# mohammadasim98/mv-ldm

Hardware: AMD Instinct MI355X
Metric: denoised views/sec @ 256x256, 4 views, 50 DDIM steps (higher is better)
Workload: dtype bf16

## Files before the change

include/mvldm.h:

```cpp
#ifndef MVLDM_H
#define MVLDM_H

#include <stddef.h>
#include <stdint.h>

#ifdef __cplusplus
extern "C" {
#endif

#define MVLDM_ABI_VERSION 7

typedef void* mvldm_stream_t;

enum { MVLDM_F32 = 0, MVLDM_BF16 = 1, MVLDM_F16 = 2 };
enum { MVLDM_OK = 0, MVLDM_ERR_ARG = -1, MVLDM_ERR_HIP = -2, MVLDM_ERR_UNSUPPORTED = -3 };

enum { MVLDM_EPI_NONE = 0, MVLDM_EPI_SILU = 1, MVLDM_EPI_GEGLU = 2, MVLDM_EPI_GELU = 3  };
enum { MVLDM_ELT_COPY = 0, MVLDM_ELT_SILU = 1, MVLDM_ELT_GELU = 2 };

int mvldm_abi_version(void);
int mvldm_build_flags(void);
const char* mvldm_last_error(void);
int mvldm_device_info(int* cu_count, size_t* hbm_bytes, char* arch, int arch_len);

typedef struct mvldm_igemm_desc {
    const void* src0;
    const void* src1;
    const void* weight;
    const float* bias;
    const float* row_bias;
    const void* residual;
    void* dst;
    float* workspace;
    int32_t c0, c1;
    int32_t n_img, h_in, w_in, h_out, w_out;
    int32_t ksize, stride, pad, upsample;
    int32_t n_out, n_pad, k_pad;
    int32_t row_bias_ld;
    int32_t epilogue;
    int32_t act_dtype;
    int32_t dst_dtype;
    int32_t splitk;
    int32_t tile;
    int32_t k_order;
    int32_t dst_ld;
    float out_scale;
    size_t workspace_bytes;
} mvldm_igemm_desc;
int mvldm_igemm_fwd(const mvldm_igemm_desc* d, mvldm_stream_t stream);
size_t mvldm_igemm_workspace_bytes(const mvldm_igemm_desc* d);

int mvldm_pack_weight(const float* src, void* dst, int n_out, int c_in, int ksize, int c_pad, int n_pad,
                      int k_pad, int geglu, int k_order, int dst_dtype, int transpose, int c_off, int n_rows,
                      mvldm_stream_t stream);

int mvldm_pack_skinny(const void* packed, void* dst, int n_pad, int k_pad, int geglu, int dtype, mvldm_stream_t stream);
int mvldm_igemm_skinny_config(const mvldm_igemm_desc* d);

typedef struct mvldm_pack_job {
    const float* src; void* dst;
    int n_out, c_in, ksize, c_pad, n_pad, k_pad, geglu, k_order, transpose, c_off, n_rows;
    int kind;
    int blocks;
    int block0;
} mvldm_pack_job;
int mvldm_pack_job_prepare(mvldm_pack_job* job , int dst_dtype);
int mvldm_pack_weight_batch(const mvldm_pack_job* jobs , int n_jobs, const int32_t* block_job, int total_blocks,
                            int dst_dtype, mvldm_stream_t stream);

#define MVLDM_GN_MAX_CHUNKS 32
int mvldm_groupnorm_fwd(const void* x0, const void* x1, void* y, const float* gamma, const float* beta, int n_img,
                        int hw, int c0, int c1, int groups, float eps, int silu, int dtype, void* stats_ws,
                        float* stats_out, mvldm_stream_t stream);
int mvldm_groupnorm_passes(int n_img, int hw, int c, int groups, int dtype);

int mvldm_layernorm_fwd(const void* x, void* y, const float* gamma, const float* beta, int rows, int c, float eps,
                        int dtype, mvldm_stream_t stream);

int mvldm_attention_fwd(const void* q, const void* k, const void* v, void* out, int ld_q, int ld_k, int ld_v,
                        int ld_o, int heads, int head_dim, const int32_t* seg, int n_seg, int max_q_len,
                        float scale, int dtype, float* lse, int lse_ld, mvldm_stream_t stream);

int mvldm_timestep_embed_fwd(const int64_t* timesteps, const float* freqs, void* out, int n, int dim,
                             int flip_sin_to_cos, int dst_dtype, mvldm_stream_t stream);

int mvldm_eltwise_fwd(const void* x, void* y, size_t n, int op, int src_dtype, int dst_dtype, mvldm_stream_t stream);

int mvldm_ddim_cfg_step(const float* eps, const float* x_t, float* x_next, const int32_t* cond_img,
                        const int32_t* uncond_img, int n_tgt, int hw, int c, float cfg_scale, const float* coef,
                        const int32_t* step_ptr, void* unet_in, int unet_in_c, int unet_in_dtype, int n_steps,
                        float clip_range, mvldm_stream_t stream);
int mvldm_ddpm_cfg_step(const float* eps_c, const float* eps_u, const float* x_t, const float* noise, float* x_next, size_t n,
                        float cfg_scale, const float* coef, float clip_range, mvldm_stream_t stream);
int mvldm_ddim_advance(int32_t* step_ptr, const int64_t* t_table, int n_steps, int64_t* timesteps,
                       const int32_t* tgt_rows, int n_rows, mvldm_stream_t stream);

int mvldm_nchw_to_nhwc(const float* src, void* dst, int n_img, int c, int hw, int dst_c, int dst_c_off,
                       int dst_dtype, float scale, float shift, const int32_t* img_map, mvldm_stream_t stream);
int mvldm_nhwc_to_nchw(const void* src, float* dst, int n_img, int c, int hw, int src_c, int src_c_off,
                       int src_dtype, float scale, float shift, int clamp01, mvldm_stream_t stream);

enum { MVLDM_RAYS_RAW = 0, MVLDM_RAYS_POSITIONAL = 1, MVLDM_RAYS_SRT = 2 };
int mvldm_ray_channels(int mode, int n_origin_octaves, int n_dir_octaves);
int mvldm_ray_encode(const float* extrinsics, const float* intrinsics, int n_cam, int h, int w, float* out_nchw,
                     void* out_nhwc, int nhwc_c, int nhwc_c_off, int nhwc_dtype, const int32_t* img_map, int mode,
                     int n_origin_octaves, int n_dir_octaves, int plucker, mvldm_stream_t stream);

int mvldm_posterior_sample(const float* moments, const float* noise, float* out, int n, int c, int hw, float scale,
                           mvldm_stream_t stream);


typedef struct mvldm_wgrad_desc {
    const void* src0; const void* src1; const void* dy;
    float* grad;
    float* workspace; size_t workspace_bytes;
    int32_t c0, c1, c_in;
    int32_t n_img, h_in, w_in, h_out, w_out;
    int32_t ksize, stride, pad, upsample;
    int32_t n_out, dy_ld;
    int32_t act_dtype;
    int32_t accumulate;
} mvldm_wgrad_desc;
int mvldm_igemm_wgrad(const mvldm_wgrad_desc* d, mvldm_stream_t stream);

int mvldm_colsum(const void* x, float* dst, float* workspace, size_t workspace_bytes, int n_seg, int rows_per_seg, int n,
                 int ld, int ld_dst, int per_seg, int accumulate, int dtype, mvldm_stream_t stream);

#define MVLDM_NORM_BWD_STORE 0x100
int mvldm_groupnorm_bwd(const void* x0, const void* x1, const void* dy, void* dx0, void* dx1, const float* gamma,
                        const float* beta, const float* stats, float* dgamma, float* dbeta, int n_img, int hw, int c0,
                        int c1, int groups, int silu, int dtype, float* workspace, size_t workspace_bytes,
                        mvldm_stream_t stream);
int mvldm_layernorm_bwd(const void* x, const void* dy, void* dx, const float* gamma, float* dgamma, float* dbeta,
                        int rows, int c, float eps, int dtype, float* workspace, size_t workspace_bytes,
                        mvldm_stream_t stream);

typedef struct mvldm_attn_bwd_desc {
    const void* q; const void* k; const void* v; const void* out; const void* dout;
    void* dq; void* dk; void* dv;
    const float* lse; float* delta;
    const int32_t* seg;
    int32_t ld_q, ld_k, ld_v, ld_o, ld_do, ld_dq, ld_dk, ld_dv;
    int32_t heads, head_dim, n_seg, max_q_len, max_kv_len, total_q_rows, stat_ld, dtype;
    float scale;
} mvldm_attn_bwd_desc;
int mvldm_attention_bwd(const mvldm_attn_bwd_desc* d, mvldm_stream_t stream);

enum { MVLDM_TE_SILU_BWD = 0, MVLDM_TE_ADD = 1, MVLDM_TE_GEGLU_FWD = 2, MVLDM_TE_GEGLU_BWD = 3, MVLDM_TE_GELU_BWD = 4 };
int mvldm_train_eltwise(int op, const void* a, const void* b, void* out, size_t rows, int d, int a_dtype, int dtype,
                        mvldm_stream_t stream);
int mvldm_pool2x2_sum(const void* du, void* dx, int n_img, int h, int w, int c, int dtype, mvldm_stream_t stream);
int mvldm_zero_insert2x(const void* x, void* out, int n_img, int h, int w, int c, int dtype, mvldm_stream_t stream);

int mvldm_add_noise(const float* x0, const float* noise, const float* coef, void* dst, int n, int c, int hw, int dst_c,
                    int dst_c_off, int dst_dtype, const int32_t* img_map, mvldm_stream_t stream);
int mvldm_mse_loss(const float* pred, const float* noise, const int32_t* tgt_img, int n_tgt, int hw, int c, float* loss,
                   int accumulate, float loss_scale, void* dpred, int dpred_c, int dpred_dtype, float grad_scale,
                   double* workspace, mvldm_stream_t stream);

typedef struct mvldm_amp_state {
    float scale;
    int32_t growth_tracker;
    int32_t adam_step;
    int32_t found_inf;
    int32_t skipped;
    int32_t reserved[3];
} mvldm_amp_state;
int mvldm_mse_loss_amp(const float* pred, const float* noise, const int32_t* tgt_img, int n_tgt, int hw, int c, float* loss,
                       int accumulate, float loss_scale, void* dpred, int dpred_c, int dpred_dtype, float grad_scale,
                       const float* amp_scale, double* workspace, mvldm_stream_t stream);

int mvldm_grad_norm(const float* g, size_t n, const float* sumsq_in, float max_norm, float* norm_out, double* workspace,
                    mvldm_stream_t stream);
int mvldm_adamw_step(float* p, const float* g, float* m, float* v, size_t n, float lr, float beta1, float beta2, float eps,
                     float weight_decay, int step, float grad_scale, const float* clip, mvldm_stream_t stream);
int mvldm_grad_norm_amp(const float* g, size_t n, const float* sumsq_in, float max_norm, float* norm_out, mvldm_amp_state* amp,
                        double* workspace, mvldm_stream_t stream);
int mvldm_adamw_step_amp(float* p, const float* g, float* m, float* v, size_t n, float lr, float beta1, float beta2, float eps,
                         float weight_decay, float grad_scale, const float* clip, const mvldm_amp_state* amp, mvldm_stream_t stream);
int mvldm_amp_update(mvldm_amp_state* amp, float growth_factor, float backoff_factor, int growth_interval, mvldm_stream_t stream);

int mvldm_ema_update(float* avg, const float* p, size_t n, float weight, mvldm_stream_t stream);

int mvldm_gather_rows(const void* src, void* dst, const int32_t* src_index, const int32_t* dst_index, int n_rows, size_t row_bytes,
                      mvldm_stream_t stream);

int mvldm_attention_merge(const void* oa, const float* lse_a, const void* ob, const float* lse_b, void* out, const int32_t* a_img,
                          const int32_t* b_img, const int32_t* out_img, int n_img, int tokens, int heads, int head_dim, int ld_a, int ld_b,
                          int ld_o, int lse_ld_a, int lse_ld_b, int dtype, mvldm_stream_t stream);

size_t mvldm_image_metrics_workspace_bytes(int n_img, int c, int h, int w);
int mvldm_image_metrics(const float* pred, const float* gt, int n_img, int c, int h, int w, int use_sample_covariance, float* psnr,
                        float* ssim, double* workspace, size_t workspace_bytes, mvldm_stream_t stream);

size_t mvldm_lpips_workspace_bytes(int n_img, int h, int w);
int mvldm_lpips_tap_slots(int h, int w, int c);
int mvldm_lpips_prep(const float* in0, const float* in1, void* dst, int n_img, int h, int w, int c_pad, int dtype, int normalize,
                     mvldm_stream_t stream);
int mvldm_lpips_relu(void* x, size_t n, int dtype, mvldm_stream_t stream);
int mvldm_lpips_tap(const void* feat, const float* weight, void* pooled, int n_img, int h, int w, int c, int dtype, double* workspace,
                    size_t workspace_bytes, int slot0, int slots_per_image, mvldm_stream_t stream);
// ... 152 lines not shown
```

mv_ldm_amd/_build.py:

```python
from __future__ import annotations

import json
import os
import re
import subprocess
import sys
from concurrent.futures import ThreadPoolExecutor
from pathlib import Path

CSRC = Path(__file__).resolve().parent / "csrc"
LIB = CSRC / "libmvldm_hip.so"
SOURCES = ["api.cpp", "plan.cpp", "igemm.hip", "igemm_small.hip", "igemm_large.hip", "igemm_xl.hip", "igemm_halo.hip", "pack.hip", "attention.hip", "norm.hip", "misc.hip",
           "wgrad.hip", "attention_bwd.hip", "norm_bwd.hip", "train_misc.hip", "linear_pp.hip", "linear_pw.hip", "linear_ws.hip", "linear_rs.hip", "skinny.hip", "metrics.hip", "lpips.hip", "dists.hip", "fid.hip", "inception.hip", "kid.hip", "cropshim.hip", "jpeg.hip", "jpeg_host.cpp"]
HEADERS = [*sorted(CSRC.glob("*.h")), CSRC.parent.parent / "include" / "mvldm.h"]
FLAGS = ["--offload-arch=gfx950", "-O3", "-std=c++17", "-fPIC", "-ffp-contract=off", "-Wno-unused-result",
         "-Rpass-analysis=kernel-resource-usage"]
RES = CSRC / "kernel_resources.json"


def _hipcc() -> str:
    for c in (os.environ.get("HIPCC"), "/opt/rocm/bin/hipcc", "hipcc"):
        if c and (os.path.isabs(c) and os.path.exists(c) or not os.path.isabs(c)):
            return c
    raise RuntimeError("hipcc not found")


def _stale(target: Path, deps) -> bool:
    if not target.exists():
        return True
    t = target.stat().st_mtime
    return any(Path(d).stat().st_mtime > t for d in deps)


def build(force: bool = False, verbose: bool = False) -> Path:
    hipcc = _hipcc()
    flags = list(FLAGS)
    if os.environ.get("MVLDM_EXPERIMENTS") == "1":
        flags.append("-DMVLDM_EXPERIMENTS")
    objs, jobs = [], []
    for src in SOURCES:
        s = CSRC / src
        o = CSRC / (s.stem + ".o")
        objs.append(o)
        if force or _stale(o, [s, *HEADERS]):
            cmd = [hipcc, *flags, "-x", "hip", "-c", str(s), "-o", str(o)]
            jobs.append(cmd)
    if jobs:
        def run(cmd):
            if verbose:
                print(" ".join(cmd), flush=True)
            r = subprocess.run(cmd, capture_output=True, text=True)
            if r.returncode:
                raise RuntimeError(f"hipcc failed: {' '.join(cmd)}\n{r.stdout}\n{r.stderr}")
            Path(cmd[-1]).with_suffix(".res.json").write_text(json.dumps(_resources(r.stderr), indent=0))
        with ThreadPoolExecutor(max_workers=min(8, len(jobs))) as ex:
            list(ex.map(run, jobs))
    if force or jobs or _stale(LIB, objs):
        cmd = [hipcc, "--offload-arch=gfx950", "-shared", "-fPIC", "-o", str(LIB), *map(str, objs)]
        r = subprocess.run(cmd, capture_output=True, text=True)
        if r.returncode:
            raise RuntimeError(f"link failed:\n{r.stdout}\n{r.stderr}")
    parts = [o.with_suffix(".res.json") for o in objs]
    if all(q.exists() for q in parts) and (not RES.exists() or _stale(RES, parts)):
        merged = {}
        for q in parts:
            merged.update(json.loads(q.read_text()))
        RES.write_text(json.dumps(merged, indent=0, sort_keys=True))
    return LIB


_FIELDS = {"VGPRs": "vgpr", "AGPRs": "agpr", "TotalSGPRs": "sgpr", "ScratchSize [bytes/lane]": "scratch", "VGPRs Spill": "vgpr_spill",
           "Occupancy [waves/SIMD]": "waves_per_simd"}


def _resources(stderr: str) -> dict:
    out, cur = {}, None
    for line in stderr.splitlines():
        m = re.search(r"remark:\s+(.*?)\s*\[-Rpass-analysis", line)
        if not m:
            continue
        body = m.group(1)
        if body.startswith("Function Name:"):
            cur = out.setdefault(body.split(":", 1)[1].strip(), {})
        elif cur is not None and ":" in body:
            k, v = body.rsplit(":", 1)
            if k.strip() in _FIELDS and v.strip().lstrip("-").isdigit():
                cur[_FIELDS[k.strip()]] = int(v)
    return out


if __name__ == "__main__":
    print(build(force="--force" in sys.argv, verbose=True))
```

mv_ldm_amd/_lib.py:

```python
from __future__ import annotations

import ctypes as C
from pathlib import Path

LIB_PATH = Path(__file__).resolve().parent / "csrc" / "libmvldm_hip.so"

ABI_VERSION = 7
F32, BF16, F16 = 0, 1, 2
EPI_NONE, EPI_SILU, EPI_GEGLU, EPI_GELU = 0, 1, 2, 3
RAYS_RAW, RAYS_POSITIONAL, RAYS_SRT = 0, 1, 2
ELT_COPY, ELT_SILU, ELT_GELU = 0, 1, 2
NORM_BWD_STORE = 0x100
GN_MAX_CHUNKS = 32
JPEG_GRAY, JPEG_444, JPEG_422, JPEG_420 = 0, 1, 2, 3
JPEG_REASONS = ("ok", "not a JPEG", "truncated", "corrupt", "progressive", "frame type", "precision", "components", "sampling", "colour space",
                "scans", "size", "range guard")
JPEG_RANGE = 12

(OP_IGEMM, OP_GROUPNORM, OP_LAYERNORM, OP_ATTENTION, OP_TIMESTEP_EMBED, OP_ELTWISE, OP_DDIM_STEP, OP_DDIM_ADVANCE,
 OP_NCHW_TO_NHWC, OP_NHWC_TO_NCHW, OP_MEMCPY, OP_RAY_ENCODE, OP_POSTERIOR_SAMPLE,
 OP_WGRAD, OP_ATTENTION_BWD, OP_GROUPNORM_BWD, OP_LAYERNORM_BWD, OP_COLSUM, OP_TRAIN_ELTWISE, OP_POOL2X2, OP_ZERO_INSERT,
 OP_ADD_NOISE, OP_MSE_LOSS, OP_FILL_ZERO, OP_PAR_BEGIN, OP_PAR_NEXT, OP_PAR_END, OP_GATHER_ROWS, OP_ATTN_MERGE) = range(1, 30)
TE_SILU_BWD, TE_ADD, TE_GEGLU_FWD, TE_GEGLU_BWD, TE_GELU_BWD = 0, 1, 2, 3, 4

vp, i32, f32, sz = C.c_void_p, C.c_int32, C.c_float, C.c_size_t


class IgemmDesc(C.Structure):
    _fields_ = [("src0", vp), ("src1", vp), ("weight", vp), ("bias", vp), ("row_bias", vp), ("residual", vp),
                ("dst", vp), ("workspace", vp),
                ("c0", i32), ("c1", i32),
                ("n_img", i32), ("h_in", i32), ("w_in", i32), ("h_out", i32), ("w_out", i32),
                ("ksize", i32), ("stride", i32), ("pad", i32), ("upsample", i32),
                ("n_out", i32), ("n_pad", i32), ("k_pad", i32),
                ("row_bias_ld", i32), ("epilogue", i32), ("act_dtype", i32), ("dst_dtype", i32),
                ("splitk", i32), ("tile", i32), ("k_order", i32), ("dst_ld", i32), ("out_scale", f32), ("workspace_bytes", sz)]


class _GroupNorm(C.Structure):
    _fields_ = [("x", vp), ("x1", vp), ("y", vp), ("gamma", vp), ("beta", vp), ("stats_ws", vp),
                ("n_img", i32), ("hw", i32), ("c0", i32), ("c1", i32), ("groups", i32), ("silu", i32), ("dtype", i32),
                ("eps", f32), ("stats_out", vp)]


class _LayerNorm(C.Structure):
    _fields_ = [("x", vp), ("y", vp), ("gamma", vp), ("beta", vp), ("rows", i32), ("c", i32), ("dtype", i32), ("eps", f32)]


class _Attention(C.Structure):
    _fields_ = [("q", vp), ("k", vp), ("v", vp), ("out", vp), ("seg", vp),
                ("ld_q", i32), ("ld_k", i32), ("ld_v", i32), ("ld_o", i32), ("heads", i32), ("head_dim", i32),
                ("n_seg", i32), ("max_q_len", i32), ("dtype", i32), ("scale", f32), ("lse", vp), ("lse_ld", i32)]


class _Temb(C.Structure):
    _fields_ = [("timesteps", vp), ("freqs", vp), ("out", vp), ("n", i32), ("dim", i32), ("flip", i32), ("dst_dtype", i32)]


class _Eltwise(C.Structure):
    _fields_ = [("x", vp), ("y", vp), ("n", sz), ("op", i32), ("src_dtype", i32), ("dst_dtype", i32)]


class _Ddim(C.Structure):
    _fields_ = [("eps", vp), ("x_t", vp), ("x_next", vp), ("cond_img", vp), ("uncond_img", vp), ("coef", vp),
                ("step_ptr", vp), ("unet_in", vp),
                ("n_tgt", i32), ("hw", i32), ("c", i32), ("unet_in_c", i32), ("unet_in_dtype", i32), ("cfg_scale", f32),
                ("n_steps", i32), ("clip_range", f32)]


class _Advance(C.Structure):
    _fields_ = [("step_ptr", vp), ("t_table", vp), ("timesteps", vp), ("tgt_rows", vp), ("n_steps", i32), ("n_rows", i32)]


class _Layout(C.Structure):
    _fields_ = [("src", vp), ("dst", vp), ("n_img", i32), ("c", i32), ("hw", i32), ("other_c", i32),
                ("other_c_off", i32), ("dtype", i32), ("clamp01", i32), ("scale", f32), ("shift", f32), ("img_map", vp)]


class _Rays(C.Structure):
    _fields_ = [("extrinsics", vp), ("intrinsics", vp), ("out_nchw", vp), ("out_nhwc", vp), ("img_map", vp),
                ("n_cam", i32), ("h", i32), ("w", i32), ("nhwc_c", i32), ("nhwc_c_off", i32), ("nhwc_dtype", i32),
                ("mode", i32), ("n_origin_octaves", i32), ("n_dir_octaves", i32), ("plucker", i32)]


class _Posterior(C.Structure):
    _fields_ = [("moments", vp), ("noise", vp), ("out", vp), ("n", i32), ("c", i32), ("hw", i32), ("scale", f32)]


class _Memcpy(C.Structure):
    _fields_ = [("src", vp), ("dst", vp), ("bytes", sz)]


class _AttnMerge(C.Structure):
    _fields_ = [("oa", vp), ("ob", vp), ("out", vp), ("lse_a", vp), ("lse_b", vp), ("a_img", vp), ("b_img", vp), ("out_img", vp),
                ("n_img", i32), ("tokens", i32), ("heads", i32), ("head_dim", i32), ("ld_a", i32), ("ld_b", i32), ("ld_o", i32),
                ("lse_ld_a", i32), ("lse_ld_b", i32), ("dtype", i32)]


class _Gather(C.Structure):
    _fields_ = [("src", vp), ("dst", vp), ("src_index", vp), ("dst_index", vp), ("row_bytes", sz), ("n_rows", i32)]


class PackJob(C.Structure):
    _fields_ = [("src", vp), ("dst", vp), ("n_out", i32), ("c_in", i32), ("ksize", i32), ("c_pad", i32), ("n_pad", i32), ("k_pad", i32),
                ("geglu", i32), ("k_order", i32), ("transpose", i32), ("c_off", i32), ("n_rows", i32), ("kind", i32), ("blocks", i32),
                ("block0", i32)]


class WgradDesc(C.Structure):
    _fields_ = [("src0", vp), ("src1", vp), ("dy", vp), ("grad", vp), ("workspace", vp), ("workspace_bytes", sz),
                ("c0", i32), ("c1", i32), ("c_in", i32),
                ("n_img", i32), ("h_in", i32), ("w_in", i32), ("h_out", i32), ("w_out", i32),
                ("ksize", i32), ("stride", i32), ("pad", i32), ("upsample", i32),
                ("n_out", i32), ("dy_ld", i32), ("act_dtype", i32), ("accumulate", i32)]


class AttnBwdDesc(C.Structure):
    _fields_ = [("q", vp), ("k", vp), ("v", vp), ("out", vp), ("dout", vp), ("dq", vp), ("dk", vp), ("dv", vp),
                ("lse", vp), ("delta", vp), ("seg", vp),
                ("ld_q", i32), ("ld_k", i32), ("ld_v", i32), ("ld_o", i32), ("ld_do", i32), ("ld_dq", i32), ("ld_dk", i32), ("ld_dv", i32),
                ("heads", i32), ("head_dim", i32), ("n_seg", i32), ("max_q_len", i32), ("max_kv_len", i32), ("total_q_rows", i32),
                ("stat_ld", i32), ("dtype", i32), ("scale", f32)]


class _GroupNormBwd(C.Structure):
    _fields_ = [("x0", vp), ("x1", vp), ("dy", vp), ("dx0", vp), ("dx1", vp), ("gamma", vp), ("beta", vp), ("stats", vp),
                ("dgamma", vp), ("dbeta", vp), ("workspace", vp), ("workspace_bytes", sz),
                ("n_img", i32), ("hw", i32), ("c0", i32), ("c1", i32), ("groups", i32), ("silu", i32), ("dtype", i32)]


class _LayerNormBwd(C.Structure):
    _fields_ = [("x", vp), ("dy", vp), ("dx", vp), ("gamma", vp), ("dgamma", vp), ("dbeta", vp), ("workspace", vp),
                ("workspace_bytes", sz), ("rows", i32), ("c", i32), ("dtype", i32), ("eps", f32)]


class _Colsum(C.Structure):
    _fields_ = [("x", vp), ("dst", vp), ("workspace", vp), ("workspace_bytes", sz),
                ("n_seg", i32), ("rows_per_seg", i32), ("n", i32), ("ld", i32), ("ld_dst", i32), ("per_seg", i32),
                ("accumulate", i32), ("dtype", i32)]


class _TrainEltwise(C.Structure):
    _fields_ = [("a", vp), ("b", vp), ("out", vp), ("rows", sz), ("op", i32), ("d", i32), ("a_dtype", i32), ("dtype", i32)]


class _Resample(C.Structure):
    _fields_ = [("src", vp), ("dst", vp), ("n_img", i32), ("h", i32), ("w", i32), ("c", i32), ("dtype", i32)]


class _AddNoise(C.Structure):
    _fields_ = [("x0", vp), ("noise", vp), ("coef", vp), ("dst", vp), ("img_map", vp),
                ("n", i32), ("c", i32), ("hw", i32), ("dst_c", i32), ("dst_c_off", i32), ("dst_dtype", i32)]


class _Mse(C.Structure):
    _fields_ = [("pred", vp), ("noise", vp), ("tgt_img", vp), ("loss", vp), ("dpred", vp), ("workspace", vp),
                ("n_tgt", i32), ("hw", i32), ("c", i32), ("accumulate", i32), ("dpred_c", i32), ("dpred_dtype", i32),
                ("loss_scale", f32), ("grad_scale", f32), ("amp_scale", vp)]


class AmpState(C.Structure):
    _fields_ = [("scale", f32), ("growth_tracker", i32), ("adam_step", i32), ("found_inf", i32), ("skipped", i32), ("reserved", i32 * 3)]


class _Fill(C.Structure):
    _fields_ = [("dst", vp), ("bytes", sz)]
# ... 156 lines not shown
```

mv_ldm_amd/csrc/igemm.hip:

```cpp
#include <algorithm>
#include <cstdio>
#include <cstdlib>

#include "igemm_common.h"

namespace mvldm {

template <typename T> __global__ __launch_bounds__(256) void igemm_splitk_reduce(const IgemmParams p) {
    const bool geglu = p.epilogue == MVLDM_EPI_GEGLU;
    const size_t total = (size_t)p.M * p.n_dst;
    const size_t slab = (size_t)p.M * p.n_pad;
    for (size_t idx = (size_t)blockIdx.x * 256 + threadIdx.x; idx < total; idx += (size_t)gridDim.x * 256) {
        const int m = (int)(idx / p.n_dst), col = (int)(idx - (size_t)m * p.n_dst);
        float v;
        if (geglu) {
            const int nv = (col >> 5) * 64 + (col & 31), ng = nv + 32;
            float a = 0.f, g = 0.f;
            for (int s = 0; s < p.splitk; ++s) {
                a += p.ws[s * slab + (size_t)m * p.n_pad + nv];
                g += p.ws[s * slab + (size_t)m * p.n_pad + ng];
            }
            if (p.bias) { a += p.bias[col]; g += p.bias[p.n_dst + col]; }
            v = a * gelu_erf_fast(g);
        } else {
            float a = 0.f;
            for (int s = 0; s < p.splitk; ++s) a += p.ws[s * slab + (size_t)m * p.n_pad + col];
            if (p.bias) a += p.bias[col];
            if (p.row_bias) a += p.row_bias[(size_t)(m / p.hw_out) * p.row_bias_ld + col];
            if (p.epilogue == MVLDM_EPI_SILU) a = silu_f(a);
            else if (p.epilogue == MVLDM_EPI_GELU) a = gelu_erf_fast(a);
            v = a;
        }
        epilogue_store<T, true>(p, m, col, v);
    }
}

template <typename T> __global__ __launch_bounds__(256) void igemm_splitk_reduce_vec(const IgemmParams p) {
    const bool geglu = p.epilogue == MVLDM_EPI_GEGLU;
    const int cpr = p.n_dst / 8;
    const size_t total = (size_t)p.M * cpr;
    const size_t slab = (size_t)p.M * p.n_pad;
    for (size_t idx = (size_t)blockIdx.x * 256 + threadIdx.x; idx < total; idx += (size_t)gridDim.x * 256) {
        const int m = (int)(idx / cpr), col = (int)(idx - (size_t)m * cpr) * 8;
        const int nv = geglu ? (col >> 5) * 64 + (col & 31) : col;
        const float* w0 = p.ws + (size_t)m * p.n_pad + nv;
        float a[8], g[8];
#pragma unroll
        for (int e = 0; e < 8; ++e) a[e] = g[e] = 0.f;
        int s = 0;
        for (; s + 4 <= p.splitk; s += 4) {
            f32x4 lo[4], hi[4], gl[4], gh[4];
#pragma unroll
            for (int u = 0; u < 4; ++u) {
                lo[u] = *reinterpret_cast<const f32x4*>(w0 + (s + u) * slab);
                hi[u] = *reinterpret_cast<const f32x4*>(w0 + (s + u) * slab + 4);
                if (geglu) {
                    gl[u] = *reinterpret_cast<const f32x4*>(w0 + (s + u) * slab + 32);
                    gh[u] = *reinterpret_cast<const f32x4*>(w0 + (s + u) * slab + 36);
                }
            }
#pragma unroll
            for (int u = 0; u < 4; ++u) {
#pragma unroll
                for (int e = 0; e < 4; ++e) { a[e] += lo[u][e]; a[4 + e] += hi[u][e]; }
                if (geglu) {
#pragma unroll
                    for (int e = 0; e < 4; ++e) { g[e] += gl[u][e]; g[4 + e] += gh[u][e]; }
                }
            }
        }
        for (; s < p.splitk; ++s) {
            const f32x4 lo = *reinterpret_cast<const f32x4*>(w0 + s * slab), hi = *reinterpret_cast<const f32x4*>(w0 + s * slab + 4);
#pragma unroll
            for (int e = 0; e < 4; ++e) { a[e] += lo[e]; a[4 + e] += hi[e]; }
            if (geglu) {
                const f32x4 gl = *reinterpret_cast<const f32x4*>(w0 + s * slab + 32), gh = *reinterpret_cast<const f32x4*>(w0 + s * slab + 36);
#pragma unroll
                for (int e = 0; e < 4; ++e) { g[e] += gl[e]; g[4 + e] += gh[e]; }
            }
        }
        if (p.bias) {
#pragma unroll
            for (int e = 0; e < 8; ++e) a[e] += p.bias[col + e];
        }
        if (geglu) {
#pragma unroll
            for (int e = 0; e < 8; ++e) a[e] *= gelu_erf_fast(g[e] + (p.bias ? p.bias[p.n_dst + col + e] : 0.f));
        } else {
            if (p.row_bias) {
                const float* rb = p.row_bias + (size_t)(m / p.hw_out) * p.row_bias_ld + col;
#pragma unroll
                for (int e = 0; e < 8; ++e) a[e] += rb[e];
            }
            if (p.epilogue == MVLDM_EPI_SILU) {
#pragma unroll
                for (int e = 0; e < 8; ++e) a[e] = silu_f(a[e]);
            } else if (p.epilogue == MVLDM_EPI_GELU) {
#pragma unroll
                for (int e = 0; e < 8; ++e) a[e] = gelu_erf_fast(a[e]);
            }
        }
#pragma unroll
        for (int e = 0; e < 8; ++e) a[e] *= p.out_scale;
        if (p.residual) {
            const Chunk<T> rc = load_chunk<T>(reinterpret_cast<const T*>(p.residual) + (size_t)m * p.n_dst + col);
#pragma unroll
            for (int e = 0; e < 8; ++e) a[e] += rc.get(e);
        }
        size_t drow = (size_t)m;
        if (p.scatter) {
            const int img = m / p.hw_out, rem = m - img * p.hw_out;
            const int i = rem / p.w_out, j = rem - i * p.w_out;
            drow = ((size_t)img * (2 * p.h_out) + 2 * i + p.ph_y) * (size_t)(2 * p.w_out) + 2 * j + p.ph_x;
        }
        Chunk<T> oc;
#pragma unroll
        for (int e = 0; e < 8; ++e) oc.set(e, a[e]);
        store_chunk<T>(reinterpret_cast<T*>(p.dst) + drow * p.dst_ld + col, oc);
    }
}

static int env_int(const char* name, int dflt) { return knob_int(name, dflt); }
static const int kEnvTarget = env_int("MVLDM_IGEMM_TARGET", 0);
static const int kEnvSync = env_int("MVLDM_IGEMM_SYNC", 0);
static const int kEnvPx = env_int("MVLDM_IGEMM_PX", 0);
static const int kEnvNoStage = env_int("MVLDM_IGEMM_NOSTAGE", 0);
#ifdef MVLDM_EXPERIMENTS
static const int kEnvFake = env_int("MVLDM_IGEMM_FAKE", 0);
#else
static constexpr int kEnvFake = 0;
#endif

static thread_local int t_force_sync = 0;

static int launch_igemm(const IgemmParams& p, int tile, int act_dtype, hipStream_t s) {
    if (tile >= 1 && tile <= 5) return igemm_launch_small(p, tile, act_dtype, s);
    if (tile >= 6 && tile <= 8) return igemm_launch_large(p, tile, act_dtype, s);
    if (tile == 9 || tile == 10 || tile == 18) return igemm_launch_xl(p, tile, act_dtype, s);
    if (tile == 11 || tile == 17) return igemm_launch_halo(p, tile, act_dtype, s);
    return set_error(MVLDM_ERR_ARG, "igemm: bad tile %d", tile);
}


static void choose_config(const mvldm_igemm_desc& d, int M, int k_tiles, int& tile, int& splitk, size_t ws_bytes) {
    const int target = kEnvTarget ? kEnvTarget : 512;
    if (tile == 0) {
        const bool can10 = d.act_dtype != MVLDM_F32 && d.k_order == 1 && d.dst_dtype != MVLDM_F32 && d.n_pad % 320 == 0 &&
                           d.epilogue != MVLDM_EPI_GEGLU && d.upsample != 1 && d.n_out % 8 == 0 && (d.dst_ld <= 0 || d.dst_ld % 8 == 0) &&
                           !(d.ksize == 3 && d.src1);
        const int wgs10 = cdiv(M, 256) * (d.n_pad / 320);
        const double eff10 = (double)wgs10 / (256.0 * cdiv(wgs10, 256));
        if (can10 && (wgs10 >= 1024 || (wgs10 >= 512 && (eff10 >= 0.9 || d.ksize == 1)))) tile = 10;
        else if (M <= 32) tile = 5;
        else if (M <= 64) tile = 4;
        else if (d.ksize >= 2) tile = cdiv(M, 256) * cdiv(d.n_pad, 128) >= 300 ? 7 : 2;
        else if (d.n_pad >= 768 && d.act_dtype != MVLDM_F32 && d.k_order == 1 && d.dst_dtype != MVLDM_F32 &&
                 cdiv(M, 256) * cdiv(d.n_pad, 256) >= 1024)
            tile = 9;
        else if (d.k_pad >= 1024 && d.n_pad >= 1024 && cdiv(M, 128) * cdiv(d.n_pad, 256) >= 300) tile = 8;
        else tile = d.n_pad < 640 ? 2 : 3;
    }
    const int tm = cdiv(M, kTiles[tile].bm), tn = cdiv(d.n_pad, kTiles[tile].bn);
    if (splitk == 0) {
        splitk = 1;
        const int wgs = tm * tn;
        if (wgs < target) splitk = std::min(std::max(k_tiles / 4, 1), cdiv(target, wgs));
        if (d.workspace == nullptr) splitk = 1;
        while (splitk > 1 && (size_t)splitk * M * d.n_pad * sizeof(float) > ws_bytes) --splitk;
    }
    splitk = std::max(1, std::min(splitk, k_tiles));
}

static int fill_params(const mvldm_igemm_desc& d, IgemmParams& p, int& tile) {
    const int epc = d.act_dtype == MVLDM_F32 ? 4 : 8;
    const int bk = d.act_dtype == MVLDM_F32 ? 32 : 64;
    MVLDM_REQUIRE(d.src0 && d.weight && d.dst, "igemm: null pointer");
    const bool phase = d.upsample >= 2;
    MVLDM_REQUIRE(d.upsample >= 0 && d.upsample <= 5, "igemm: upsample %d", d.upsample);
    MVLDM_REQUIRE(phase ? (d.ksize == 2 && d.stride == 1 && d.h_out == d.h_in && d.w_out == d.w_in && !d.src1 && !d.residual &&
                           !d.row_bias && d.act_dtype != MVLDM_F32 && d.dst_dtype == d.act_dtype && d.k_order == 1)
                        : (d.ksize == 1 || d.ksize == 3),
                  "igemm: ksize %d / upsample %d", d.ksize, d.upsample);
    MVLDM_REQUIRE(d.stride == 1 || d.stride == 2, "igemm: stride %d", d.stride);
    MVLDM_REQUIRE(d.c0 % epc == 0 && d.c1 % epc == 0 && d.c0 > 0, "igemm: channels (%d,%d) must be multiples of %d", d.c0, d.c1, epc);
    MVLDM_REQUIRE((d.c1 == 0) == (d.src1 == nullptr), "igemm: src1/c1 mismatch");
    MVLDM_REQUIRE(d.k_pad % bk == 0 && d.k_pad >= d.ksize * d.ksize * (d.c0 + d.c1), "igemm: k_pad %d", d.k_pad);
    MVLDM_REQUIRE(d.n_pad % 64 == 0 && d.n_pad >= d.n_out, "igemm: n_pad %d (n_out %d)", d.n_pad, d.n_out);
    MVLDM_REQUIRE(d.dst_dtype == d.act_dtype || d.dst_dtype == MVLDM_F32, "igemm: dst dtype");
    if (d.epilogue == MVLDM_EPI_GEGLU)
        MVLDM_REQUIRE(d.n_out % 64 == 0 && !d.row_bias, "igemm: GEGLU needs n_out %% 64 == 0");
    p.src0 = d.src0; p.src1 = d.src1; p.weight = d.weight; p.bias = d.bias; p.row_bias = d.row_bias;
    p.residual = d.residual; p.dst = d.dst; p.ws = d.workspace;
    p.c0 = d.c0; p.c1 = d.c1; p.ctot = d.c0 + d.c1;
    p.n_img = d.n_img; p.h_in = d.h_in; p.w_in = d.w_in; p.h_out = d.h_out; p.w_out = d.w_out;
    p.hw_out = d.h_out * d.w_out;
    p.ksize = d.ksize; p.stride = d.stride; p.pad = d.pad; p.upsample = phase ? 0 : d.upsample; p.taps = d.ksize * d.ksize;
    p.scatter = phase; p.ph_y = phase ? (d.upsample - 2) >> 1 : 0; p.ph_x = phase ? (d.upsample - 2) & 1 : 0;
    p.ty0 = phase ? p.ph_y - 1 : -d.pad; p.tx0 = phase ? p.ph_x - 1 : -d.pad;
    p.cy = phase ? 1 - p.ph_y : d.ksize / 2; p.cx = phase ? 1 - p.ph_x : d.ksize / 2;
    p.M = d.n_img * p.hw_out; p.n_out = d.n_out; p.n_pad = d.n_pad; p.k_pad = d.k_pad;
    p.n_dst = d.epilogue == MVLDM_EPI_GEGLU ? d.n_out / 2 : d.n_out;
    p.rb_vec = d.row_bias && ((uintptr_t)d.row_bias % 16 == 0) && d.row_bias_ld % 4 == 0;
    p.bias_vec = d.bias && ((uintptr_t)d.bias % 16 == 0);
    p.row_bias_ld = d.row_bias_ld; p.epilogue = d.epilogue; p.dst_f32 = d.dst_dtype == MVLDM_F32;
    p.out_scale = d.out_scale;
    p.dst_ld = d.dst_ld > 0 ? d.dst_ld : p.n_dst;
    MVLDM_REQUIRE(p.dst_ld >= p.n_dst, "igemm: dst_ld %d < n_dst %d", p.dst_ld, p.n_dst);
    p.k_tiles = d.k_pad / bk;
    tile = d.tile & 63;
    t_force_sync = (d.tile >> 12) & 1;
    const int force_px = (d.tile >> 8) & 15;
    int splitk = d.splitk;
    MVLDM_REQUIRE(((tile >= 0 && tile <= kNumTiles) || tile == 17 || deep_tile(tile)) && splitk >= 0, "igemm: tile/splitk");
    choose_config(d, p.M, p.k_tiles, tile, splitk, d.workspace_bytes);
    if (splitk > 1)
        MVLDM_REQUIRE(d.workspace && (size_t)splitk * p.M * d.n_pad * sizeof(float) <= d.workspace_bytes,
                      "igemm: split-K workspace too small");
    const double es = 2.0;
    const double b0 = (double)d.n_img * d.h_in * d.w_in * d.c0 * es, b1 = (double)d.n_img * d.h_in * d.w_in * d.c1 * es;
    const double bw = (double)d.n_pad * d.k_pad * es;
    p.use_bl = d.act_dtype != MVLDM_F32 && d.k_order == 1 && !t_force_sync && !kEnvSync &&
               b0 < 4.0e9 && b1 < 4.0e9 && bw < 4.0e9;
    if (d.act_dtype != MVLDM_F32 && d.k_order == 1 && !t_force_sync && !kEnvSync && !p.use_bl) {
        static bool warned = false;
        if (!warned) {
            warned = true;
            fprintf(stderr, "[mvldm] igemm: operand of %.2f GB exceeds the 4 GB range of the fast 16-bit loop; using the slower "
                            "64-bit-address loop (split the batch to avoid this)\n", std::max(std::max(b0, b1), bw) / 1e9);
        }
    }
    p.src0_bytes = (unsigned)b0; p.src1_bytes = (unsigned)b1; p.w_bytes = (unsigned)bw;
    p.fake = kEnvFake;
    p.nt_store = stream_stores((size_t)p.M * (size_t)p.n_dst * (p.dst_f32 || d.act_dtype == MVLDM_F32 ? 4 : 2));
    if (kEnvFake & 1) p.src0_bytes = p.src1_bytes = 0;
    if (kEnvFake & 2) p.w_bytes = 0;
    if (tile >= 6 && !p.use_bl) tile = 2;
    if (deep_tile(tile) && d.upsample) tile = 2;
    p.splitk = splitk;
    if (p.use_bl) {
        const int cbs = p.k_tiles / p.taps;
        const int per = cdiv(cbs, std::min(splitk, cbs));
        p.k_tiles_per_split = per * p.taps;
        p.splitk = cdiv(cbs, per);
    } else {
        p.k_tiles_per_split = cdiv(p.k_tiles, splitk);
        p.splitk = cdiv(p.k_tiles, p.k_tiles_per_split);
    }
    p.stage_epi = d.act_dtype != MVLDM_F32 && !kEnvNoStage && (p.splitk > 1 || (!p.dst_f32 && p.n_dst % 8 == 0 && p.dst_ld % 8 == 0));
    if (tile >= 9 && tile <= 10 && (!p.stage_epi || (tile == 10 && d.epilogue == MVLDM_EPI_GEGLU))) tile = 7;
    if (tile == 11 && !(p.use_bl && p.stage_epi && p.splitk == 1 && d.ksize == 3 && d.stride == 1 && d.pad == 1 && !d.upsample &&
                        d.h_out == d.h_in && d.w_out == d.w_in && halo_rows_for(d.w_in) <= 384 && halo_smem(d.w_in) <= 160 * 1024))
        tile = 7;
    if (tile == 17 && !(p.use_bl && p.stage_epi && p.splitk == 1 && d.ksize == 3 && d.stride == 1 && d.pad == 1 && !d.upsample && d.c1 == 0 &&
                        d.h_out == d.h_in && d.w_out == d.w_in && d.epilogue != MVLDM_EPI_GEGLU && halow_smem(d.w_in) <= 160 * 1024))
        tile = 7;
    if (phase) {
        MVLDM_REQUIRE(p.use_bl && p.stage_epi, "igemm: 2x2 phase conv needs the lean 16-bit loop and an 8-aligned 16-bit output");
        if (tile != 7 && tile != 10) tile = 2;
    }
    if (p.use_bl && d.upsample == 1 && tile != 7) tile = 2;
    if (p.use_bl && d.upsample != 1) {
        const int hc = (d.h_out - 1) * d.stride + p.ty0 + p.cy, wc = (d.w_out - 1) * d.stride + p.tx0 + p.cx;
        MVLDM_REQUIRE(p.ty0 + p.cy >= 0 && p.tx0 + p.cx >= 0 && hc < d.h_in && wc < d.w_in,
                      "igemm: conv geometry (pad %d, stride %d) not supported", d.pad, d.stride);
    }
    p.tiles_m = cdiv(p.M, kTiles[tile].bm);
    p.tiles_n = cdiv(d.n_pad, kTiles[tile].bn);
    p.korder = d.k_order;
    if (d.k_order)
        MVLDM_REQUIRE(d.k_order == 1 && p.ctot % bk == 0 && d.c0 % bk == 0 && d.k_pad == p.taps * p.ctot,
                      "igemm: k_order 1 needs channel counts (%d,%d) multiples of %d", d.c0, d.c1, bk);
    {
        const double a_bytes = (double)d.n_img * d.h_in * d.w_in * p.ctot, w_bytes = (double)d.n_pad * d.k_pad;
        double best = 1e300;
        for (int px = 1; px <= 8; px *= 2) {
            const int py = 8 / px;
            const int sm = cdiv(p.tiles_m, px), sn = cdiv(p.tiles_n, py);
            const double waste = (double)(8 * sm * sn) / ((double)p.tiles_m * p.tiles_n);
            const double cost = (py * a_bytes + px * w_bytes) * waste * waste;
            if (cost < best) { best = cost; p.px = px; p.sub_m = sm; p.sub_n = sn; }
        }
        p.m_fast = w_bytes >= a_bytes;
        const int fpx = force_px ? force_px : kEnvPx;
        if (fpx > 0 && fpx <= 8 && (8 % fpx) == 0) {
            p.px = fpx; p.sub_m = cdiv(p.tiles_m, p.px); p.sub_n = cdiv(p.tiles_n, 8 / p.px);
        }
        p.grp_m = p.grp_n = 1;
        static const int kGroup = knob_int("MVLDM_IGEMM_GROUP", -1);
        if (kGroup != 0 && ((tile >= 7 && tile <= 10) || tile == 17) && p.sub_m * p.sub_n > 32) {
            const double ax = a_bytes / p.px, wx = w_bytes / (8 / p.px);
            double bestc = 1e300;
            for (int gm = 1; gm <= 32; gm *= 2) {
                if (kGroup > 0 && gm != kGroup) continue;
                const int gme = std::min(gm, p.sub_m), gne = std::min(32 / gm, p.sub_n);
                const double c = ax * cdiv(p.sub_n, gne) + wx * cdiv(p.sub_m, gme);
                if (c < bestc) { bestc = c; p.grp_m = gme; p.grp_n = gne; }
            }
        }
    }
    return MVLDM_OK;
}

int linear_pp_run(const mvldm_igemm_desc& d, hipStream_t s);
int linear_pw_run(const mvldm_igemm_desc& d, hipStream_t s);
int linear_ws_run(const mvldm_igemm_desc& d, hipStream_t s);
int skinny_run(const mvldm_igemm_desc& d, hipStream_t s);
int linear_rs_run(const mvldm_igemm_desc& d, hipStream_t s);

int igemm_run(const mvldm_igemm_desc& d, hipStream_t s) {
    IgemmParams p;
    int tile = 0;
    if (d.n_img == 0 || d.h_out == 0 || d.w_out == 0) return MVLDM_OK;
    const int req = d.tile & 63;
    if (req == 15) return skinny_run(d, s);
    if (req == 12 || req == 13 || req == 14 || req == 19) {
        MVLDM_REQUIRE(d.src0 && d.weight && d.dst, "igemm: null pointer");
        return req == 12 ? linear_pp_run(d, s) : req == 13 ? linear_pw_run(d, s) : req == 14 ? linear_ws_run(d, s) : linear_rs_run(d, s);
    }
    MVLDM_REQUIRE(d.k_order != 2, "igemm: the fragment-order pack (k_order 2) is read by tile 15 only");
    int rc = fill_params(d, p, tile);
    if (rc) return rc;
    if (p.M == 0) return MVLDM_OK;
    rc = dispatch_dtype(d.act_dtype, [&](auto t) {
        using T = decltype(t);
        int r = launch_igemm(p, tile, Elt<T>::DT, s);
        if (r) return r;
        if (p.splitk > 1) {
            if constexpr (sizeof(T) == 2) {
                if (!p.dst_f32 && p.n_dst % 8 == 0 && p.dst_ld % 8 == 0 && ((uintptr_t)p.ws % 16) == 0 &&
                    (!p.residual || ((uintptr_t)p.residual % 16) == 0) && ((uintptr_t)p.dst % 16) == 0) {
                    const size_t chunks = (size_t)p.M * (p.n_dst / 8);
                    hipLaunchKernelGGL(igemm_splitk_reduce_vec<T>, dim3((unsigned)std::min<size_t>((chunks + 255) / 256, 4096)), dim3(256), 0, s, p);
                    return check_launch();
                }
            }
            const size_t total = (size_t)p.M * p.n_dst;
            const int blocks = (int)std::min<size_t>((total + 255) / 256, 4096);
            hipLaunchKernelGGL(igemm_splitk_reduce<T>, dim3(blocks), dim3(256), 0, s, p);
            return check_launch();
        }
        return (int)MVLDM_OK;
    });
    return rc;
}

}

using namespace mvldm;

extern "C" int mvldm_igemm_fwd(const mvldm_igemm_desc* d, mvldm_stream_t stream) {
    MVLDM_REQUIRE(d != nullptr, "igemm: null desc");
    return igemm_run(*d, (hipStream_t)stream);
}

extern "C" size_t mvldm_igemm_workspace_bytes(const mvldm_igemm_desc* d) {
    if (!d) return 0;
    const size_t M = (size_t)d->n_img * d->h_out * d->w_out;
    return (size_t)16 * M * d->n_pad * sizeof(float);
}
```

mv_ldm_amd/csrc/igemm_bl.h:

```cpp
#pragma once
#include "igemm_common.h"

namespace mvldm {

template <typename T, int BM, int BN, int WM, int WN>
__global__ __launch_bounds__(WM* WN * 64) void igemm_kernel(const IgemmParams p) {
    using M_ = Mma<T>;
    constexpr int NT = WM * WN * 64;
    constexpr int EPC = Elt<T>::EPC;
    constexpr int BK = M_::BK;
    constexpr int TM = BM / WM / 32, TN = BN / WN / 32;
    constexpr int A_BYTES = BM * M_::PITCH, B_BYTES = BN * M_::PITCH;
    constexpr int A_IT = BM * 8 / NT, B_IT = BN * 8 / NT;
    static_assert(A_IT >= 1 && B_IT >= 1 && TM >= 1 && TN >= 1, "bad tile");
    extern __shared__ __attribute__((aligned(16))) char smem[];

    const int tid = threadIdx.x, lane = tid & 63, wave = tid >> 6;
    const int wm = wave / WN, wn = wave % WN;
    const int hi = lane >> 5, l31 = lane & 31;

    int split, tm, tn;
    if (!map_block(p, split, tm, tn)) return;
    const int kt0 = split * p.k_tiles_per_split;
    const int kt1 = min(kt0 + p.k_tiles_per_split, p.k_tiles);
// ... 31 lines not shown
        const bool tap_ok = tap < p.taps;
        const int ky = tap / p.ksize, kx = tap - ky * p.ksize;
        const bool from0 = c < p.c0;
        const T* sbase = from0 ? reinterpret_cast<const T*>(p.src0) + c
                               : reinterpret_cast<const T*>(p.src1) + (c - p.c0);
        const int cs = from0 ? p.c0 : p.c1;
#pragma unroll
        for (int it = 0; it < A_IT; ++it) {
            int iy = a_y[it] + ky, ix = a_x[it] + kx;
            const bool ok = tap_ok && a_img[it] >= 0 && iy >= 0 && iy < hs && ix >= 0 && ix < wsz;
            if (p.upsample) { iy >>= 1; ix >>= 1; }
            if (ok) {
                const size_t off = ((size_t)(a_img[it] * p.h_in + iy) * p.w_in + ix) * cs;
                areg[it] = *reinterpret_cast<const u32x4*>(sbase + off);
            } else {
                areg[it] = u32x4{0u, 0u, 0u, 0u};
            }
        }
#pragma unroll
        for (int it = 0; it < B_IT; ++it) {
            const int n = tn * BN + r0 + it * (NT / 8);
            if (n < p.n_pad)
                breg[it] = *reinterpret_cast<const u32x4*>(wbase + (size_t)it * (NT / 8) * p.k_pad + (size_t)kt * BK);
            else
                breg[it] = u32x4{0u, 0u, 0u, 0u};
        }
    };
    auto store_tile = [&](int stage) {
        char* at = smem + stage * (A_BYTES + B_BYTES);
        char* bt = at + A_BYTES;
#pragma unroll
        for (int it = 0; it < A_IT; ++it) M_::store(at, r0 + it * (NT / 8), kc, areg[it]);
#pragma unroll
        for (int it = 0; it < B_IT; ++it) M_::store(bt, r0 + it * (NT / 8), kc, breg[it]);
    };

    f32x16 acc[TM][TN];
#pragma unroll
    for (int i = 0; i < TM; ++i)
#pragma unroll
        for (int j = 0; j < TN; ++j)
#pragma unroll
            for (int r = 0; r < 16; ++r) acc[i][j][r] = 0.f;

    if (kt0 < kt1) {
        load_tile(kt0);
        store_tile(0);
    }
    __syncthreads();
    int cur = 0;
    for (int kt = kt0; kt < kt1; ++kt) {
        const bool more = kt + 1 < kt1;
        if (more) load_tile(kt + 1);
        const char* at = smem + cur * (A_BYTES + B_BYTES);
        const char* bt = at + A_BYTES;
#pragma unroll
        for (int kk = 0; kk < BK / M_::KI; ++kk) {
            typename M_::Frag a[TM], b[TN];
#pragma unroll
            for (int i = 0; i < TM; ++i) a[i] = M_::load(at, wm * (BM / WM) + i * 32 + l31, kk, hi);
#pragma unroll
            for (int j = 0; j < TN; ++j) b[j] = M_::load(bt, wn * (BN / WN) + j * 32 + l31, kk, hi);
#pragma unroll
            for (int i = 0; i < TM; ++i)
#pragma unroll
                for (int j = 0; j < TN; ++j) acc[i][j] = M_::mma(a[i], b[j], acc[i][j]);
        }
        if (more) store_tile(cur ^ 1);
        __syncthreads();
        cur ^= 1;
    }

    if constexpr (sizeof(T) == 2) {
        if (p.stage_epi) {
            igemm_epilogue_staged<T, BM, BN, WM, WN>(p, acc, tm, tn, split, wm, wn, wave, lane, smem);
            return;
        }
    }
    igemm_epilogue<T, BM, BN, WM, WN>(p, acc, tm, tn, split, wm, wn, hi, l31);
}


template <int TAPS, int A_IT, bool DUAL, bool UPS> struct BlAddr {
    unsigned a0[UPS ? TAPS : 1][A_IT];
    unsigned a1[DUAL ? (UPS ? TAPS : 1) : 1][DUAL ? A_IT : 1];
    unsigned mask[UPS ? 1 : A_IT];
};

template <typename T, int BM, int BN, int NW, int KS, bool DUAL, int A_IT, int B_IT, int STAGES, bool UPS, int t, int LO = 0, int HI = 1 << 20>
__device__ __forceinline__ void bl_issue(const IgemmParams& p, char* stage_base, int wave, int cb,
                                         const BlAddr<KS * KS, A_IT, DUAL, UPS>& ad, const unsigned (&vb)[B_IT]) {
    constexpr int BK = 64, TAPS = KS * KS;
    const int lead = (!UPS && KS > 1) ? p.w_in + 1 : 0;
    const int disp = UPS ? 0 : (t / KS - p.cy) * p.w_in + (t % KS - p.cx) + lead;
    const unsigned lead0 = (unsigned)lead * (unsigned)p.c0 * 2u, lead1 = (unsigned)lead * (unsigned)p.c1 * 2u;
    const __amdgpu_buffer_rsrc_t r0 = __builtin_amdgcn_make_buffer_rsrc(
        const_cast<char*>(reinterpret_cast<const char*>(p.src0)) - lead0, 0, p.src0_bytes + lead0, 0x00020000);
    const __amdgpu_buffer_rsrc_t r1 = __builtin_amdgcn_make_buffer_rsrc(
        const_cast<char*>(reinterpret_cast<const char*>(DUAL ? p.src1 : p.src0)) - (DUAL ? lead1 : lead0), 0,
        DUAL ? p.src1_bytes + lead1 : p.src0_bytes + lead0, 0x00020000);
    const __amdgpu_buffer_rsrc_t rw = __builtin_amdgcn_make_buffer_rsrc(const_cast<void*>(p.weight), 0, p.w_bytes, 0x00020000);
    char* at = stage_base;
    char* bt = at + BM * 128;
    const int c = cb * BK;
    const bool from0 = !DUAL || c < p.c0;
    const int soff = ((from0 ? c : c - p.c0) + disp * (from0 ? p.c0 : p.c1)) * 2;
#pragma unroll
    for (int it = (LO > 0 ? LO : 0); it < (HI < A_IT ? HI : A_IT); ++it) {
        __attribute__((address_space(3))) void* dst = (__attribute__((address_space(3))) void*)(at + (wave + NW * it) * 1024);
        unsigned v0, v1;
        if constexpr (UPS) {
            v0 = ad.a0[t][it];
            v1 = ad.a1[DUAL ? t : 0][DUAL ? it : 0];
        } else {
            const bool ok = (ad.mask[it] >> t) & 1u;
            v0 = ok ? ad.a0[0][it] : kBufOob;
            v1 = ok ? ad.a1[0][DUAL ? it : 0] : kBufOob;
        }
        if (from0) __builtin_amdgcn_raw_ptr_buffer_load_lds(r0, dst, 16, v0, soff, 0, 0);
        else __builtin_amdgcn_raw_ptr_buffer_load_lds(r1, dst, 16, v1, soff, 0, 0);
    }
    const int koff = (cb * TAPS + t) * (BK * 2);
#pragma unroll
    for (int it = (LO > A_IT ? LO - A_IT : 0); it < (HI - A_IT < B_IT ? HI - A_IT : B_IT); ++it)
        __builtin_amdgcn_raw_ptr_buffer_load_lds(rw, (__attribute__((address_space(3))) void*)(bt + (wave + NW * it) * 1024), 16,
                                                 vb[it], koff, 0, 0);
}

template <typename T, int BM, int BN, int WM, int WN>
__device__ __forceinline__ void bl_compute(const char* stage_base, f32x16 (&acc)[BM / WM / 32][BN / WN / 32], int wm, int wn,
                                           int hi, int l31) {
    constexpr int TM = BM / WM / 32, TN = BN / WN / 32;
#pragma unroll
    for (int kk = 0; kk < 64 / Mma<T>::KI; ++kk) {
        BlFrags<T, TM, TN> f;
        bl_load<T, BM, BN, WM, WN>(stage_base, f, kk, wm, wn, hi, l31);
        bl_mma<T, TM, TN>(f, acc);
    }
}

template <int LPT, int MAXY>
__device__ __forceinline__ void bl_wait_young(int young) {
    if constexpr (MAXY >= 1) {
        if (young >= MAXY) {
            asm volatile("s_waitcnt vmcnt(%0) lgkmcnt(0)" ::"n"(MAXY * LPT) : "memory");
            return;
        }
        bl_wait_young<LPT, MAXY - 1>(young);
    } else {
        asm volatile("s_waitcnt vmcnt(0) lgkmcnt(0)" ::: "memory");
    }
}

template <typename T, int BM, int BN, int WM, int WN, int KS, bool DUAL, int STAGES, bool UPS>
__global__ __launch_bounds__(WM* WN * 64) void igemm_bl_kernel(const IgemmParams p) {
    using M_ = Mma<T>;
    static_assert(sizeof(T) == 2, "16-bit activation types only");
    constexpr int NW = WM * WN, TAPS = KS * KS;
    constexpr int BK = 64, EPC = 8;
    constexpr int TM = BM / WM / 32, TN = BN / WN / 32;
    constexpr int A_BYTES = BM * 128, B_BYTES = BN * 128, STAGE_BYTES = A_BYTES + B_BYTES;
    constexpr int A_IT = BM / 8 / NW, B_IT = BN / 8 / NW, LPT = A_IT + B_IT;
    static_assert(A_IT >= 1 && B_IT >= 1 && (BM / 8) % NW == 0 && (BN / 8) % NW == 0, "bad tile");
    static_assert(STAGES >= 2 && STAGES <= 8, "ring depth");
    extern __shared__ __attribute__((aligned(16))) char smem[];

    const auto [lane, wave, wm, wn, hi, l31] = wave_lane<WN>();
    int split, tm, tn;
    if (!map_block(p, split, tm, tn)) return;
    const int cb0 = split * (p.k_tiles_per_split / TAPS);
    const int cb1 = min(cb0 + p.k_tiles_per_split / TAPS, p.k_tiles / TAPS);

    const int slot = lane & 7, rsub = lane >> 3;
    BlAddr<TAPS, A_IT, DUAL, UPS> ad;
#pragma unroll
    for (int it = 0; it < A_IT; ++it) {
        const int row = (wave + NW * it) * 8 + rsub;
        const int m = tm * BM + row;
        const unsigned chunk = (unsigned)((slot ^ ((row >> 1) & 7)) * EPC);
        const bool live = m < p.M;
        const int img = live ? m / p.hw_out : 0, rem = live ? m - img * p.hw_out : 0;
        const int oy = rem / p.w_out, ox = rem - oy * p.w_out;
        if constexpr (UPS) {
            const unsigned hs = 2 * p.h_in, wsz = 2 * p.w_in;
            const int y0 = live ? oy * p.stride - p.pad : -(1 << 20), x0 = ox * p.stride - p.pad;
#pragma unroll
            for (int t = 0; t < TAPS; ++t) {
                const int iy = y0 + t / KS, ix = x0 + t % KS;
                const bool ok = (unsigned)iy < hs && (unsigned)ix < wsz;
                const unsigned pix = (unsigned)(img * p.h_in + (iy >> 1)) * (unsigned)p.w_in + (unsigned)(ix >> 1);
                ad.a0[t][it] = ok ? (pix * (unsigned)p.c0 + chunk) * 2u : kBufOob;
                if constexpr (DUAL) ad.a1[t][it] = ok ? (pix * (unsigned)p.c1 + chunk) * 2u : kBufOob;
            }
        } else {
            const int yc = oy * p.stride + p.ty0 + p.cy, xc = ox * p.stride + p.tx0 + p.cx;
            const unsigned pix = (unsigned)(img * p.h_in + yc) * (unsigned)p.w_in + (unsigned)xc;
            unsigned msk = 0;
#pragma unroll
            for (int t = 0; t < TAPS; ++t) {
                const int iy = yc + t / KS - p.cy, ix = xc + t % KS - p.cx;
                msk |= (live && (unsigned)iy < (unsigned)p.h_in && (unsigned)ix < (unsigned)p.w_in) ? (1u << t) : 0u;
            }
            ad.a0[0][it] = (pix * (unsigned)p.c0 + chunk) * 2u;
            if constexpr (DUAL) ad.a1[0][it] = (pix * (unsigned)p.c1 + chunk) * 2u;
            ad.mask[it] = msk;
        }
    }
    unsigned vb[B_IT];
#pragma unroll
    for (int it = 0; it < B_IT; ++it) {
        const int row = (wave + NW * it) * 8 + rsub;
        const int n = tn * BN + row;
        const unsigned chunk = (unsigned)((slot ^ ((row >> 1) & 7)) * EPC);
        vb[it] = n < p.n_pad ? ((unsigned)n * (unsigned)p.k_pad + chunk) * 2u : kBufOob;
    }

    f32x16 acc[TM][TN];
#pragma unroll
    for (int i = 0; i < TM; ++i)
#pragma unroll
        for (int j = 0; j < TN; ++j)
#pragma unroll
            for (int r = 0; r < 16; ++r) acc[i][j][r] = 0.f;

#define MVLDM_BL_ISSUE(stage_, cb_, t_) \
    bl_issue<T, BM, BN, NW, KS, DUAL, A_IT, B_IT, STAGES, UPS, t_>(p, smem + (stage_) * STAGE_BYTES, wave, cb_, ad, vb)
#define MVLDM_BL_ISSUE_R(stage_, cb_, t_, lo_, hi_) \
    bl_issue<T, BM, BN, NW, KS, DUAL, A_IT, B_IT, STAGES, UPS, t_, lo_, hi_>(p, smem + (stage_) * STAGE_BYTES, wave, cb_, ad, vb)
#define MVLDM_BL_NEXT(t_, d_) (((t_) + (d_)) % TAPS)
#define MVLDM_BL_LOAD(f_, slot_, kk_) bl_load<T, BM, BN, WM, WN>(smem + (slot_) * STAGE_BYTES, f_, kk_, wm, wn, hi, l31)
#define MVLDM_BL_MMA(f_)                  \
    __builtin_amdgcn_sched_barrier(0);    \
    bl_mma<T, TM, TN>(f_, acc);           \
    __builtin_amdgcn_sched_barrier(0);
#define MVLDM_BL_STEP(t_)                                                                                         \
    {                                                                                                             \
        static_assert(64 / M_::KI == 4, "four k-sub-steps per K-tile");                                          \
        MVLDM_BL_LOAD(f1, slot_c, 1);                                                                             \
        MVLDM_BL_MMA(f0)                                                                                          \
        MVLDM_BL_LOAD(f0, slot_c, 2);                                                                             \
        MVLDM_BL_MMA(f1)                                                                                          \
        MVLDM_BL_LOAD(f1, slot_c, 3);                                                                             \
        MVLDM_BL_MMA(f0)                                                                                          \
            \
                             \
        if (STAGES == 3 && cb + ((t_) + 2) / TAPS < cb1) asm volatile("s_waitcnt vmcnt(%0) lgkmcnt(0)" ::"n"(LPT) : "memory"); \
        else asm volatile("s_waitcnt vmcnt(0) lgkmcnt(0)" ::: "memory");                                          \
        __builtin_amdgcn_s_barrier();                                                                             \
        {                                                                                                         \
                   \
            const int cbn_ = cb + ((t_) + STAGES) / TAPS;                                                         \
            if (cbn_ < cb1) { MVLDM_BL_ISSUE(slot_c, cbn_, MVLDM_BL_NEXT(t_, STAGES)); }                          \
        }                                                                                                         \
        slot_c = slot_c + 1 == STAGES ? 0 : slot_c + 1;                                                           \
        MVLDM_BL_LOAD(f0, slot_c, 0);                                                                             \
        MVLDM_BL_MMA(f1)                                                                                          \
    }
#ifdef MVLDM_BL_BURST
    constexpr bool SPREAD_S = false;
#elif defined(MVLDM_BL_SPREAD_ALL)
    constexpr bool SPREAD_S = true;
#else
    constexpr bool SPREAD_S = NW == 8;
#endif
#define MVLDM_BL_STEP_SIMPLE(t_)                                                                                  \
    {                                                                                                             \
        asm volatile("s_waitcnt vmcnt(0) lgkmcnt(0)" ::: "memory");                                               \
        __builtin_amdgcn_s_barrier();                                                                             \
        if constexpr (!SPREAD_S) {                                                                                \
            const int cbn_ = cb + ((t_) + 1) / TAPS;                                                              \
            if (cbn_ < cb1) { MVLDM_BL_ISSUE(slot_c ^ 1, cbn_, MVLDM_BL_NEXT(t_, 1)); }                           \
            bl_compute<T, BM, BN, WM, WN>(smem + slot_c * STAGE_BYTES, acc, wm, wn, hi, l31);                     \
        } else {                                                                                                  \
            constexpr int Q0_ = (4 * LPT + 8) / 9, Q1_ = Q0_ + (LPT - Q0_ + 1) / 2;                              \
            const int cbn_ = cb + ((t_) + 1) / TAPS;                                                              \
            const bool more_ = cbn_ < cb1;                                                                        \
            if (more_) { MVLDM_BL_ISSUE_R(slot_c ^ 1, cbn_, MVLDM_BL_NEXT(t_, 1), 0, Q0_); }                      \
            {                                                                                                     \
                BlFrags<T, TM, TN> fs_;                                                                           \
                MVLDM_BL_LOAD(fs_, slot_c, 0);                                                                    \
                bl_mma<T, TM, TN>(fs_, acc);                                                                      \
            }                                                                                                     \
            if (more_) { MVLDM_BL_ISSUE_R(slot_c ^ 1, cbn_, MVLDM_BL_NEXT(t_, 1), Q0_, Q1_); }                    \
            {                                                                                                     \
                BlFrags<T, TM, TN> fs_;                                                                           \
                MVLDM_BL_LOAD(fs_, slot_c, 1);                                                                    \
                bl_mma<T, TM, TN>(fs_, acc);                                                                      \
            }                                                                                                     \
            if (more_) { MVLDM_BL_ISSUE_R(slot_c ^ 1, cbn_, MVLDM_BL_NEXT(t_, 1), Q1_, LPT); }                    \
            {                                                                                                     \
                BlFrags<T, TM, TN> fs_;                                                                           \
                MVLDM_BL_LOAD(fs_, slot_c, 2);                                                                    \
                bl_mma<T, TM, TN>(fs_, acc);                                                                      \
                MVLDM_BL_LOAD(fs_, slot_c, 3);                                                                    \
                bl_mma<T, TM, TN>(fs_, acc);                                                                      \
            }                                                                                                     \
        }                                                                                                         \
        slot_c ^= 1;                                                                                              \
    }
#define MVLDM_BL_STEP_DEEP(t_)                                                                                    \
    {                                                                                                             \
        bl_wait_young<LPT, STAGES - 2>((cb1 - cb) * TAPS - (t_) - 1);       \
        __builtin_amdgcn_s_barrier();                                       \
        {                                                                                                         \
            const int cbn_ = cb + ((t_) + STAGES - 1) / TAPS;                                                     \
            if (cbn_ < cb1) { MVLDM_BL_ISSUE(slot_c == 0 ? STAGES - 1 : slot_c - 1, cbn_, MVLDM_BL_NEXT(t_, STAGES - 1)); } \
        }                                                                                                         \
        bl_compute<T, BM, BN, WM, WN>(smem + slot_c * STAGE_BYTES, acc, wm, wn, hi, l31);                         \
        slot_c = slot_c + 1 == STAGES ? 0 : slot_c + 1;                                                           \
    }
#define MVLDM_BL_PRO(j_)                                                                                          \
    if constexpr (STAGES - 1 > (j_)) {                                                                            \
        if (cb0 + (j_) / TAPS < cb1) { MVLDM_BL_ISSUE((j_), cb0 + (j_) / TAPS, ((j_) % TAPS)); }                  \
    }
    constexpr bool PIPE = NW == 8 && TM * TN <= 8 && STAGES <= 3;
    if constexpr (STAGES > 3) {
        static_assert((STAGES - 2) * LPT <= 63, "vmcnt is a 6-bit counter");
        if (cb0 < cb1) {
            MVLDM_BL_ISSUE(0, cb0, 0);
            MVLDM_BL_PRO(1) MVLDM_BL_PRO(2) MVLDM_BL_PRO(3) MVLDM_BL_PRO(4) MVLDM_BL_PRO(5) MVLDM_BL_PRO(6)
            int slot_c = 0;
            for (int cb = cb0; cb < cb1; ++cb) {
                MVLDM_BL_STEP_DEEP(0)
                if constexpr (TAPS == 4) { MVLDM_BL_STEP_DEEP(1) MVLDM_BL_STEP_DEEP(2) MVLDM_BL_STEP_DEEP(3) }
                if constexpr (TAPS == 9) {
                    MVLDM_BL_STEP_DEEP(1) MVLDM_BL_STEP_DEEP(2) MVLDM_BL_STEP_DEEP(3) MVLDM_BL_STEP_DEEP(4)
                    MVLDM_BL_STEP_DEEP(5) MVLDM_BL_STEP_DEEP(6) MVLDM_BL_STEP_DEEP(7) MVLDM_BL_STEP_DEEP(8)
                }
            }
        }
    } else if constexpr (!PIPE) {
        static_assert(STAGES == 2, "the plain loop uses the 2-slot ring");
        if (cb0 < cb1) {
            MVLDM_BL_ISSUE(0, cb0, 0);
            int slot_c = 0;
            for (int cb = cb0; cb < cb1; ++cb) {
                MVLDM_BL_STEP_SIMPLE(0)
                if constexpr (TAPS == 4) { MVLDM_BL_STEP_SIMPLE(1) MVLDM_BL_STEP_SIMPLE(2) MVLDM_BL_STEP_SIMPLE(3) }
                if constexpr (TAPS == 9) {
                    MVLDM_BL_STEP_SIMPLE(1) MVLDM_BL_STEP_SIMPLE(2) MVLDM_BL_STEP_SIMPLE(3) MVLDM_BL_STEP_SIMPLE(4)
                    MVLDM_BL_STEP_SIMPLE(5) MVLDM_BL_STEP_SIMPLE(6) MVLDM_BL_STEP_SIMPLE(7) MVLDM_BL_STEP_SIMPLE(8)
                }
            }
        }
    } else if (cb0 < cb1) {
        MVLDM_BL_ISSUE(0, cb0, 0);
        const bool has1 = cb0 + 1 / TAPS < cb1, has2 = STAGES == 3 && cb0 + 2 / TAPS < cb1;
        if (has1) { MVLDM_BL_ISSUE(1, cb0 + 1 / TAPS, (1 % TAPS)); }
        if constexpr (STAGES == 3) {
            if (has2) { MVLDM_BL_ISSUE(2, cb0 + 2 / TAPS, (2 % TAPS)); }
        }
        if (has2) asm volatile("s_waitcnt vmcnt(%0)" ::"n"(2 * LPT) : "memory");
        else if (has1) asm volatile("s_waitcnt vmcnt(%0)" ::"n"(LPT) : "memory");
        else asm volatile("s_waitcnt vmcnt(0)" ::: "memory");
        __builtin_amdgcn_s_barrier();
        int slot_c = 0;
        BlFrags<T, TM, TN> f0, f1;
        MVLDM_BL_LOAD(f0, 0, 0);
        for (int cb = cb0; cb < cb1; ++cb) {
            MVLDM_BL_STEP(0)
            if constexpr (TAPS == 4) { MVLDM_BL_STEP(1) MVLDM_BL_STEP(2) MVLDM_BL_STEP(3) }
            if constexpr (TAPS == 9) {
                MVLDM_BL_STEP(1) MVLDM_BL_STEP(2) MVLDM_BL_STEP(3) MVLDM_BL_STEP(4)
                MVLDM_BL_STEP(5) MVLDM_BL_STEP(6) MVLDM_BL_STEP(7) MVLDM_BL_STEP(8)
            }
        }
    }
#undef MVLDM_BL_STEP_SIMPLE
#undef MVLDM_BL_STEP_DEEP
#undef MVLDM_BL_PRO
#undef MVLDM_BL_LOAD
#undef MVLDM_BL_MMA
#undef MVLDM_BL_NEXT
#undef MVLDM_BL_STEP
#undef MVLDM_BL_ISSUE
#undef MVLDM_BL_ISSUE_R
    asm volatile("s_waitcnt vmcnt(0)" ::: "memory");
    if constexpr (TM * TN > 4) {
        igemm_epilogue_staged<T, BM, BN, WM, WN>(p, acc, tm, tn, split, wm, wn, wave, lane, smem);
    } else {
        if (p.stage_epi) igemm_epilogue_staged<T, BM, BN, WM, WN>(p, acc, tm, tn, split, wm, wn, wave, lane, smem);
        else igemm_epilogue<T, BM, BN, WM, WN>(p, acc, tm, tn, split, wm, wn, hi, l31);
    }
}

template <typename T, int BM, int BN, int WM, int WN> static int launch_sync(const IgemmParams& p, hipStream_t s) {
    static std::atomic<uint64_t> done{0};
    constexpr int ring = 2 * (BM + BN) * Mma<T>::PITCH, park = WM * WN * 32 * (park_blocks(BN / WN / 32) * 32 + 4) * 4;
    return launch_kernel(igemm_kernel<T, BM, BN, WM, WN>, done, (sizeof(T) == 2 && park > ring) ? park : ring,
                         8 * p.sub_m * p.sub_n * p.splitk, WM * WN * 64, p, s);
}

template <typename T, int BM, int BN, int WM, int WN, int KS, bool DUAL, int STAGES, bool UPS>
static int launch_bl_s(const IgemmParams& p, hipStream_t s) {
    static std::atomic<uint64_t> done{0};
    constexpr int ring = STAGES * (BM + BN) * 128, park = WM * WN * 32 * (park_blocks(BN / WN / 32) * 32 + 4) * 4;
    return launch_kernel(igemm_bl_kernel<T, BM, BN, WM, WN, KS, DUAL, STAGES, UPS>, done, ring > park ? ring : park,
                         8 * p.sub_m * p.sub_n * p.splitk, WM * WN * 64, p, s);
}
template <typename T, int BM, int BN, int WM, int WN, int KS, bool DUAL, int DEPTH = 0>
static int launch_bl(const IgemmParams& p, hipStream_t s) {
    constexpr int STAGES = DEPTH ? DEPTH : ((WM * WN == 8 && 3 * (BM + BN) * 128 <= 160 * 1024) ? 3 : 2);
    if (p.upsample) {
        if constexpr (KS == 3 && !DUAL && ((BM == 128 && BN == 64) || (BM == 256 && BN == 128)))
            return launch_bl_s<T, BM, BN, WM, WN, KS, DUAL, STAGES, true>(p, s);
        else
            return set_error(MVLDM_ERR_ARG, "igemm: upsampling 3x3 conv needs tile 2 or 7 on the 16-bit path");
    }
    return launch_bl_s<T, BM, BN, WM, WN, KS, DUAL, STAGES, false>(p, s);
}
template <typename T, int BM, int BN, int WM, int WN, int DEPTH> static int launch_bl_deep(const IgemmParams& p, hipStream_t s) {
    const bool dual = p.c1 > 0;
    if (p.ksize == 3) return dual ? launch_bl<T, BM, BN, WM, WN, 3, true, DEPTH>(p, s) : launch_bl<T, BM, BN, WM, WN, 3, false, DEPTH>(p, s);
    if (p.ksize == 1) return dual ? launch_bl<T, BM, BN, WM, WN, 1, true, DEPTH>(p, s) : launch_bl<T, BM, BN, WM, WN, 1, false, DEPTH>(p, s);
    return set_error(MVLDM_ERR_ARG, "igemm: the deep-ring tiles take 1x1 and 3x3 convs");
}

template <typename T, int BM, int BN, int WM, int WN> static int launch_bl_any(const IgemmParams& p, hipStream_t s) {
    const bool dual = p.c1 > 0;
    if (p.ksize == 2) {
        if constexpr ((BM == 128 && BN == 64) || (BM == 256 && BN == 128) || (BM == 256 && BN == 320))
            return launch_bl<T, BM, BN, WM, WN, 2, false>(p, s);
        else
            return set_error(MVLDM_ERR_ARG, "igemm: 2x2 phase conv needs tile 2, 7 or 10");
    }
    if (p.ksize == 3) {
        if (!dual) return launch_bl<T, BM, BN, WM, WN, 3, false>(p, s);
        if constexpr (BM == 256 && BN >= 256)
            return set_error(MVLDM_ERR_UNSUPPORTED, "igemm: tiles 9 / 10 do not take a two-source 3x3 conv (use tile 7 or 11)");
        else
            return launch_bl<T, BM, BN, WM, WN, 3, true>(p, s);
    }
    return dual ? launch_bl<T, BM, BN, WM, WN, 1, true>(p, s) : launch_bl<T, BM, BN, WM, WN, 1, false>(p, s);
}

template <typename T, int BM, int BN, int WM, int WN> static int launch_tile(const IgemmParams& p, hipStream_t s) {
    if constexpr (sizeof(T) == 2) {
        if (p.use_bl) return launch_bl_any<T, BM, BN, WM, WN>(p, s);
    }
    return launch_sync<T, BM, BN, WM, WN>(p, s);
}

}
```

mv_ldm_amd/csrc/igemm_common.h:

```cpp
#pragma once
#include <algorithm>

#include "common.h"

namespace mvldm {

struct IgemmParams {
    const void* src0; const void* src1; const void* weight;
    const float* bias; const float* row_bias; const void* residual; void* dst; float* ws;
    int c0, c1, ctot;
    int n_img, h_in, w_in, h_out, w_out, hw_out;
    int ksize, stride, pad, upsample;
    int M, n_out, n_pad, n_dst, k_pad, taps;
    int row_bias_ld, epilogue, dst_f32, dst_ld;
    float out_scale;
    int splitk, k_tiles, k_tiles_per_split;
    int tiles_m, tiles_n;
    int korder;
    int px, sub_m, sub_n, m_fast;
    int grp_m, grp_n;
    int rb_vec;
    int bias_vec;
    int ty0, tx0, cy, cx;
    int scatter, ph_y, ph_x;
    int fake;
    unsigned src0_bytes, src1_bytes, w_bytes;
    int use_bl, stage_epi;
    int nt_store;
};

template <typename T> struct Mma;

template <typename T16> struct Mma16 : Mfma16<T16> {
    static constexpr int KI = 16;
    static constexpr int BK = 64;
    static constexpr int PITCH = 128;
    using Frag = typename Mfma16<T16>::Frag;
    static __device__ __forceinline__ void store(char* tile, int r, int kc, u32x4 v) {
        *reinterpret_cast<u32x4*>(tile + r * PITCH + ((kc ^ ((r >> 1) & 7)) << 4)) = v;
    }
    static __device__ __forceinline__ Frag load(const char* tile, int r, int kk, int hi) {
        const int kc = kk * 2 + hi;
        return *reinterpret_cast<const Frag*>(tile + r * PITCH + ((kc ^ ((r >> 1) & 7)) << 4));
    }
};
template <> struct Mma<bf16_t> : Mma16<bf16_t> {};
template <> struct Mma<f16_t> : Mma16<f16_t> {};
template <> struct Mma<float> {
    static constexpr int KI = 2;
    static constexpr int BK = 32;
    static constexpr int PITCH = 33 * 4;
    using Frag = float;
    static __device__ __forceinline__ void store(char* tile, int r, int kc, u32x4 v) {
        uint32_t* p = reinterpret_cast<uint32_t*>(tile + r * PITCH + kc * 16);
        p[0] = v[0]; p[1] = v[1]; p[2] = v[2]; p[3] = v[3];
    }
    static __device__ __forceinline__ Frag load(const char* tile, int r, int kk, int hi) {
        return *reinterpret_cast<const float*>(tile + r * PITCH + (kk * 2 + hi) * 4);
    }
    static __device__ __forceinline__ f32x16 mma(Frag a, Frag b, f32x16 c) {
        return __builtin_amdgcn_mfma_f32_32x32x2f32(a, b, c, 0, 0, 0);
    }
};

__device__ __forceinline__ int orig_col(int n_packed, int n_out, bool geglu) {
    if (!geglu) return n_packed;
    const int blk = n_packed >> 5, w = n_packed & 31;
    return (blk & 1) ? (n_out >> 1) + (blk >> 1) * 32 + w : (blk >> 1) * 32 + w;
}

template <typename T, bool SCATTER = false>
__device__ __forceinline__ void epilogue_store(const IgemmParams& p, int m, int n_dst_col, float v) {
    v *= p.out_scale;
    if (p.residual) v += to_f32<T>(reinterpret_cast<const T*>(p.residual)[(size_t)m * p.n_dst + n_dst_col]);
    size_t drow = (size_t)m;
    if (SCATTER && p.scatter) {
        const int img = m / p.hw_out, rem = m - img * p.hw_out;
        const int i = rem / p.w_out, j = rem - i * p.w_out;
        drow = ((size_t)img * (2 * p.h_out) + 2 * i + p.ph_y) * (size_t)(2 * p.w_out) + 2 * j + p.ph_x;
    }
    const size_t o = drow * p.dst_ld + n_dst_col;
    if (p.dst_f32) reinterpret_cast<float*>(p.dst)[o] = v;
    else reinterpret_cast<T*>(p.dst)[o] = from_f32<T>(v);
}

__device__ __forceinline__ bool map_block(const IgemmParams& p, int& split, int& tm, int& tn) {
    const int b = blockIdx.x, xcd = b & 7, idx = b >> 3;
    const int xm = xcd % p.px, xn = xcd / p.px;
    const int per = p.sub_m * p.sub_n;
    split = idx / per;
    const int r = idx - split * per;
    int tml, tnl;
    if (p.grp_m * p.grp_n > 1) {
        const int gm = p.grp_m, gn = p.grp_n;
        const int nfull = p.sub_m / gm, per_super = gm * p.sub_n;
        int mg, gm_eff, rr;
        if (r < nfull * per_super) { mg = r / per_super; rr = r - mg * per_super; gm_eff = gm; }
        else { mg = nfull; rr = r - nfull * per_super; gm_eff = p.sub_m - nfull * gm; }
        const int ng = rr / (gm_eff * gn), r2 = rr - ng * gm_eff * gn;
        tnl = ng * gn + r2 / gm_eff;
        tml = mg * gm + r2 % gm_eff;
    } else if (p.m_fast) { tnl = r / p.sub_m; tml = r - tnl * p.sub_m; }
    else { tml = r / p.sub_n; tnl = r - tml * p.sub_n; }
    tm = xm * p.sub_m + tml;
    tn = xn * p.sub_n + tnl;
    return tm < p.tiles_m && tn < p.tiles_n;
}

template <typename T, int BM, int BN, int WM, int WN>
__device__ __forceinline__ void igemm_epilogue(const IgemmParams& p, f32x16 (&acc)[BM / WM / 32][BN / WN / 32], int tm, int tn,
                                               int split, int wm, int wn, int hi, int l31) {
    constexpr int TM = BM / WM / 32, TN = BN / WN / 32;
    const bool geglu = p.epilogue == MVLDM_EPI_GEGLU;
    if (p.splitk > 1) {
        float* ws = p.ws + (size_t)split * p.M * p.n_pad;
#pragma unroll
        for (int i = 0; i < TM; ++i)
#pragma unroll
            for (int j = 0; j < TN; ++j) {
                const int n = tn * BN + wn * (BN / WN) + j * 32 + l31;
#pragma unroll
                for (int r = 0; r < 16; ++r) {
                    const int m = tm * BM + wm * (BM / WM) + i * 32 + (r & 3) + 8 * (r >> 2) + 4 * hi;
                    if (m < p.M && n < p.n_pad) ws[(size_t)m * p.n_pad + n] = acc[i][j][r];
                }
            }
        return;
    }
#pragma unroll
    for (int i = 0; i < TM; ++i) {
        if (geglu) {
            if constexpr (TN % 2 == 0) {
#pragma unroll
                for (int j = 0; j < TN; j += 2) {
                    const int nb = tn * BN + wn * (BN / WN) + j * 32;
                    const int col = (nb >> 6) * 32 + l31;
                    if (col >= p.n_dst) continue;
                    const float bv = p.bias ? p.bias[col] : 0.f;
                    const float bg = p.bias ? p.bias[p.n_dst + col] : 0.f;
#pragma unroll
                    for (int r = 0; r < 16; ++r) {
                        const int m = tm * BM + wm * (BM / WM) + i * 32 + (r & 3) + 8 * (r >> 2) + 4 * hi;
                        if (m >= p.M) continue;
                        epilogue_store<T>(p, m, col, (acc[i][j][r] + bv) * gelu_erf_fast(acc[i][j + 1][r] + bg));
                    }
                }
            }
        } else {
#pragma unroll
            for (int j = 0; j < TN; ++j) {
                const int n = tn * BN + wn * (BN / WN) + j * 32 + l31;
                if (n >= p.n_out) continue;
                const float bv = p.bias ? p.bias[n] : 0.f;
#pragma unroll
                for (int r = 0; r < 16; ++r) {
                    const int m = tm * BM + wm * (BM / WM) + i * 32 + (r & 3) + 8 * (r >> 2) + 4 * hi;
                    if (m >= p.M) continue;
                    float v = acc[i][j][r] + bv;
                    if (p.row_bias) v += p.row_bias[(size_t)(m / p.hw_out) * p.row_bias_ld + n];
                    if (p.epilogue == MVLDM_EPI_SILU) v = silu_f(v);
                    else if (p.epilogue == MVLDM_EPI_GELU) v = gelu_erf_fast(v);
                    epilogue_store<T>(p, m, n, v);
                }
            }
        }
    }
}

constexpr int park_blocks(int tn) { return tn <= 4 ? tn : 4; }

enum { EPI_PLAIN = 0, EPI_ACT_SILU = 1, EPI_PAIR_GEGLU = 2, EPI_PARTIAL = 3, EPI_ACT_GELU = 4 };

template <typename T, int JN, int MODE, int PITCH>
__device__ __forceinline__ void epi_rows(const IgemmParams& p, const float* st, int m0, int pcol0, int split, int lane) {
    constexpr bool PAIR = MODE == EPI_PAIR_GEGLU;
    constexpr int WC = PAIR ? JN * 16 : JN * 32;
    constexpr int CPR = WC / 8;
    static_assert(64 % CPR == 0 && (32 * CPR) % 64 == 0, "row-major mapping");
    constexpr int RSTEP = 64 / CPR, ITERS = 32 / RSTEP;
    const int ch = lane % CPR, row0 = lane / CPR;
    const int ncol0 = PAIR ? (pcol0 >> 1) : pcol0;
// ... 17 lines not shown
            }
        } else {
#pragma unroll
            for (int e = 0; e < 8; ++e) {
                bv[e] = p.bias[n0 + e];
                if constexpr (PAIR) bg[e] = p.bias[p.n_dst + n0 + e];
            }
        }
    }
    const bool rb_on = MODE != EPI_PARTIAL && MODE != EPI_PAIR_GEGLU && p.row_bias != nullptr;
    Chunk<T> rpre[ITERS];
    if constexpr (MODE != EPI_PARTIAL) {
        if (p.residual && !(p.fake & 4)) {
#pragma unroll
            for (int it = 0; it < ITERS; ++it) {
                const int m = m0 + row0 + it * RSTEP;
                if (m < p.M) rpre[it] = load_chunk<T>(reinterpret_cast<const T*>(p.residual) + (size_t)m * p.n_dst + n0);
            }
        }
    }
    float rbv[8];
    bool rb_pre = false;
    if (rb_on) {
        const int img0 = m0 / p.hw_out;
        rb_pre = p.rb_vec && (min(m0 + 31, p.M - 1) / p.hw_out) == img0;
        if (rb_pre) {
            const float* rb = p.row_bias + (size_t)img0 * p.row_bias_ld + n0;
            const f32x4 r0 = *reinterpret_cast<const f32x4*>(rb), r1 = *reinterpret_cast<const f32x4*>(rb + 4);
#pragma unroll
            for (int e = 0; e < 4; ++e) { rbv[e] = r0[e]; rbv[4 + e] = r1[e]; }
        }
    }
#pragma unroll
    for (int it = 0; it < ITERS; ++it) {
        const int row = row0 + it * RSTEP;
        const int m = m0 + row;
        if (m >= p.M) continue;
        const f32x4 a = *reinterpret_cast<const f32x4*>(st + row * PITCH + voff);
        const f32x4 b = *reinterpret_cast<const f32x4*>(st + row * PITCH + voff + 4);
        if constexpr (MODE == EPI_PARTIAL) {
            float* o = p.ws + (size_t)split * p.M * p.n_pad + (size_t)m * p.n_pad + n0;
            *reinterpret_cast<f32x4*>(o) = a;
            *reinterpret_cast<f32x4*>(o + 4) = b;
        } else {
            float v[8] = {a[0] + bv[0], a[1] + bv[1], a[2] + bv[2], a[3] + bv[3], b[0] + bv[4], b[1] + bv[5], b[2] + bv[6], b[3] + bv[7]};
            if constexpr (PAIR) {
                const f32x4 ga = *reinterpret_cast<const f32x4*>(st + row * PITCH + voff + 32);
                const f32x4 gb = *reinterpret_cast<const f32x4*>(st + row * PITCH + voff + 36);
#pragma unroll
                for (int e = 0; e < 4; ++e) {
                    v[e] *= gelu_erf_16(ga[e] + bg[e]);
                    v[4 + e] *= gelu_erf_16(gb[e] + bg[4 + e]);
                }
            } else {
                if (rb_on && rb_pre) {
#pragma unroll
                    for (int e = 0; e < 8; ++e) v[e] += rbv[e];
                } else if (rb_on) {
                    const float* rb = p.row_bias + (size_t)(m / p.hw_out) * p.row_bias_ld + n0;
                    if (p.rb_vec) {
                        const f32x4 r0 = *reinterpret_cast<const f32x4*>(rb), r1 = *reinterpret_cast<const f32x4*>(rb + 4);
#pragma unroll
                        for (int e = 0; e < 4; ++e) { v[e] += r0[e]; v[4 + e] += r1[e]; }
                    } else {
#pragma unroll
                        for (int e = 0; e < 8; ++e) v[e] += rb[e];
                    }
                }
                if constexpr (MODE == EPI_ACT_SILU) {
#pragma unroll
                    for (int e = 0; e < 8; ++e) v[e] = silu_f(v[e]);
                }
                if constexpr (MODE == EPI_ACT_GELU) {
#pragma unroll
                    for (int e = 0; e < 8; ++e) v[e] = gelu_erf_fast(v[e]);
                }
            }
#pragma unroll
            for (int e = 0; e < 8; ++e) v[e] *= p.out_scale;
            if (p.fake & 4) { if (v[0] == 1.2345e33f) p.ws[0] = v[1]; continue; }
            if (p.residual) {
#pragma unroll
                for (int e = 0; e < 8; ++e) v[e] += rpre[it].get(e);
            }
            Chunk<T> oc;
#pragma unroll
            for (int e = 0; e < 8; ++e) oc.set(e, v[e]);
            size_t drow = (size_t)m;
            if (p.scatter) {
                const int img = m / p.hw_out, rem = m - img * p.hw_out;
                const int i = rem / p.w_out, j = rem - i * p.w_out;
                drow = ((size_t)img * (2 * p.h_out) + 2 * i + p.ph_y) * (size_t)(2 * p.w_out) + 2 * j + p.ph_x;
            }
            T* const dptr = reinterpret_cast<T*>(p.dst) + drow * p.dst_ld + n0;
            if (p.nt_store) __builtin_nontemporal_store(oc.raw, reinterpret_cast<u32x4*>(dptr));
            else store_chunk<T>(dptr, oc);
        }
    }
}

template <int TM, int TN, int I, int J0, int JN, int PITCH>
__device__ __forceinline__ void epi_park(const f32x16 (&acc)[TM][TN], float* st, int lane) {
    const int hi = lane >> 5, l31 = lane & 31;
#pragma unroll
    for (int j = 0; j < JN; ++j)
#pragma unroll
        for (int r = 0; r < 16; ++r) st[((r & 3) + 8 * (r >> 2) + 4 * hi) * PITCH + j * 32 + l31] = acc[I][J0 + j][r];
}

template <typename T, int JN, int PITCH>
__device__ __forceinline__ void epi_group_rows(const IgemmParams& p, const float* st, int m0, int pcol0, int split, int mode, int lane) {
    if (mode == EPI_PARTIAL) epi_rows<T, JN, EPI_PARTIAL, PITCH>(p, st, m0, pcol0, split, lane);
    else if (mode == EPI_PAIR_GEGLU) {
        if constexpr (JN % 2 == 0) epi_rows<T, JN, EPI_PAIR_GEGLU, PITCH>(p, st, m0, pcol0, split, lane);
    } else if (mode == EPI_ACT_SILU) epi_rows<T, JN, EPI_ACT_SILU, PITCH>(p, st, m0, pcol0, split, lane);
    else if (mode == EPI_ACT_GELU) epi_rows<T, JN, EPI_ACT_GELU, PITCH>(p, st, m0, pcol0, split, lane);
    else epi_rows<T, JN, EPI_PLAIN, PITCH>(p, st, m0, pcol0, split, lane);
}

template <typename T, int BM, int BN, int WM, int WN, int I>
__device__ __forceinline__ void igemm_epilogue_rowblock(const IgemmParams& p, const f32x16 (&acc)[BM / WM / 32][BN / WN / 32], float* st, int tm, int tn,
                                                        int split, int wm, int wn, int mode, int lane) {
    constexpr int TM = BM / WM / 32, TN = BN / WN / 32;
    constexpr int WCOLS = BN / WN;
    constexpr int JG = park_blocks(TN);
    constexpr int PITCH = JG * 32 + 4;
    const int m0 = tm * BM + wm * (BM / WM) + I * 32;
    const int pcol0 = tn * BN + wn * WCOLS;
    epi_park<TM, TN, I, 0, JG, PITCH>(acc, st, lane);
    epi_group_rows<T, JG, PITCH>(p, st, m0, pcol0, split, mode, lane);
    if constexpr (TN > JG) {
        epi_park<TM, TN, I, JG, TN - JG, PITCH>(acc, st, lane);
        epi_group_rows<T, TN - JG, PITCH>(p, st, m0, pcol0 + JG * 32, split, mode, lane);
    }
    if constexpr (I + 1 < TM) igemm_epilogue_rowblock<T, BM, BN, WM, WN, I + 1>(p, acc, st, tm, tn, split, wm, wn, mode, lane);
}

template <typename T, int BM, int BN, int WM, int WN>
__device__ __forceinline__ void igemm_epilogue_staged(const IgemmParams& p, f32x16 (&acc)[BM / WM / 32][BN / WN / 32], int tm,
                                                      int tn, int split, int wm, int wn, int wave, int lane, char* smem) {
    constexpr int TN = BN / WN / 32;
    constexpr int JG = park_blocks(TN);
    constexpr int PITCH = JG * 32 + 4;
    static_assert(TN <= 2 * JG, "at most two park groups");
    if (p.fake & 8) return;
    float* st = reinterpret_cast<float*>(smem) + wave * (32 * PITCH);
    const int mode = p.splitk > 1 ? EPI_PARTIAL
                                  : (p.epilogue == MVLDM_EPI_GEGLU ? EPI_PAIR_GEGLU
                                     : (p.epilogue == MVLDM_EPI_SILU ? EPI_ACT_SILU : (p.epilogue == MVLDM_EPI_GELU ? EPI_ACT_GELU : EPI_PLAIN)));
    __syncthreads();
    igemm_epilogue_rowblock<T, BM, BN, WM, WN, 0>(p, acc, st, tm, tn, split, wm, wn, mode, lane);
}

struct WaveLane { int lane, wave, wm, wn, hi, l31; };
template <int WN> __device__ __forceinline__ WaveLane wave_lane() {
    const int tid = threadIdx.x, lane = tid & 63;
    const int wave = __builtin_amdgcn_readfirstlane(tid >> 6);
    return {lane, wave, wave / WN, wave % WN, lane >> 5, lane & 31};
}

template <typename T, int TM, int TN> struct BlFrags {
    typename Mma<T>::Frag a[TM], b[TN];
};

template <typename T, int BM, int BN, int WM, int WN>
__device__ __forceinline__ void bl_load(const char* stage_base, BlFrags<T, BM / WM / 32, BN / WN / 32>& f, int kk, int wm, int wn,
                                        int hi, int l31) {
    using M_ = Mma<T>;
    constexpr int TM = BM / WM / 32, TN = BN / WN / 32;
    const char* at = stage_base;
    const char* bt = at + BM * 128;
#pragma unroll
    for (int i = 0; i < TM; ++i) f.a[i] = M_::load(at, wm * (BM / WM) + i * 32 + l31, kk, hi);
#pragma unroll
    for (int j = 0; j < TN; ++j) f.b[j] = M_::load(bt, wn * (BN / WN) + j * 32 + l31, kk, hi);
}

template <typename T, int TM, int TN>
__device__ __forceinline__ void bl_mma(const BlFrags<T, TM, TN>& f, f32x16 (&acc)[TM][TN]) {
#pragma unroll
    for (int i = 0; i < TM; ++i)
#pragma unroll
        for (int j = 0; j < TN; ++j) acc[i][j] = Mma<T>::mma(f.a[i], f.b[j], acc[i][j]);
}

inline int cdiv(int a, int b) { return (a + b - 1) / b; }
struct TileCfg { int bm, bn, threads; };
constexpr TileCfg kTiles[] = {{0, 0, 0}, {128, 128, 256}, {128, 64, 256}, {64, 128, 256}, {64, 64, 128}, {32, 64, 64},
                                 {256, 64, 256},
                                 {256, 128, 512},
                                 {128, 256, 512},
                                 {256, 256, 512},
                                 {256, 320, 512},
                                 {256, 128, 512},
                                 {0, 0, 0}, {0, 0, 0}, {0, 0, 0}, {0, 0, 0},
                                 {0, 0, 0},
                                 {256, 320, 512},
                                 {192, 128, 512}};
constexpr int kNumTiles = 11;
inline bool deep_tile(int tile) { return tile == 18; }

template <typename KernT> inline int launch_kernel(KernT kern, std::atomic<uint64_t>& attr_done, int smem, int blocks, int threads,
                                                   const IgemmParams& p, hipStream_t s) {
    if (int rc0 = ensure_dyn_smem(reinterpret_cast<const void*>(kern), smem, attr_done)) return rc0;
    hipLaunchKernelGGL(kern, dim3(blocks), dim3(threads), smem, s, p);
    return check_launch();
}

inline int halo_rows_for(int w_in) { return (256 + 2 * (w_in + 1) + 7) / 8 * 8; }
inline int halo_smem(int w_in) { return 2 * halo_rows_for(w_in) * 128 + 3 * 128 * 128 + 128 + 1024; }
inline int halow_smem(int w_in) { return 2 * halo_rows_for(w_in) * 128 + 2 * 320 * 128 + 128 + 1024; }

inline int require_bl(const IgemmParams& p, int tile, int act_dtype) {
    if (act_dtype != MVLDM_F32 && p.use_bl) return MVLDM_OK;
    return set_error(MVLDM_ERR_ARG, "igemm: tile %d needs the 16-bit block-major path", tile);
}
template <typename F> inline int dispatch_16bit(int dtype, F&& f) { return dtype == MVLDM_BF16 ? f(bf16_t{}) : f(f16_t{}); }

int igemm_launch_small(const IgemmParams& p, int tile, int act_dtype, hipStream_t s);
int igemm_launch_large(const IgemmParams& p, int tile, int act_dtype, hipStream_t s);
int igemm_launch_xl(const IgemmParams& p, int tile, int act_dtype, hipStream_t s);
int igemm_launch_halo(const IgemmParams& p, int tile, int act_dtype, hipStream_t s);

}
```

mv_ldm_amd/ops.py:

```python
from __future__ import annotations

import ctypes as C
import os
from dataclasses import dataclass
from typing import NamedTuple, Optional, Sequence

import math

import numpy as np
import torch

from . import _lib as L

_DT = {torch.float32: L.F32, torch.bfloat16: L.BF16, torch.float16: L.F16}


def dt(t) -> int:
    return _DT[t if isinstance(t, torch.dtype) else t.dtype]


def epc(dtype: torch.dtype) -> int:
    return 4 if dtype == torch.float32 else 8


# ... 39 lines not shown
            and self.ksize in (1, 2, 3) and self.n_out % 4 == 0

    def skinny(self) -> torch.Tensor:
        if self._skinny is None:
            assert self.can_skinny(), "tile 15 needs a 16-bit block-major pack with channels in multiples of 64"
            out = torch.empty_like(self.data)
            L.check(L.load().mvldm_pack_skinny(self.data.data_ptr(), out.data_ptr(), self.n_pad, self.k_pad, int(self.geglu), dt(self.data), stream()))
            self._skinny = out
        return self._skinny

    def drop_skinny(self):
        if not self._skinny_pinned:
            self._skinny = None


def block_k(dtype: torch.dtype) -> int:
    return 32 if dtype == torch.float32 else 64


def pack_weight_t(w: torch.Tensor, dtype: torch.dtype, c_off: int = 0, n_rows: Optional[int] = None,
                  out: Optional[torch.Tensor] = None) -> PackedWeight:
    assert w.is_cuda and w.dtype == torch.float32 and w.is_contiguous()
    n_out, c_in = w.shape[0], w.shape[1]
    ksize = w.shape[2] if w.ndim == 4 else 1
    n_rows = c_in - c_off if n_rows is None else n_rows
    c_pad = _roundup(n_out, epc(dtype))
    bk = block_k(dtype)
    k_pad = _roundup(ksize * ksize * c_pad, bk)
    n_pad = _roundup(n_rows, 64)
    k_order = int(c_pad % bk == 0)
    data = torch.zeros(n_pad, k_pad, dtype=dtype, device=w.device) if out is None else out
    L.check(L.load().mvldm_pack_weight(w.data_ptr(), data.data_ptr(), n_out, c_in, ksize, c_pad, n_pad, k_pad, 0, k_order, dt(dtype),
                                       1, c_off, n_rows, stream()))
    return PackedWeight(data, n_rows, n_pad, k_pad, c_pad, ksize, False, k_order)


def pack_weight(w: torch.Tensor, dtype: torch.dtype, c_pad: Optional[int] = None, geglu: bool = False,
                c_split: Optional[int] = None, out: Optional[torch.Tensor] = None) -> PackedWeight:
    assert w.is_cuda, "pack_weight needs a device tensor (no CPU path)"
    w = w.detach().to(torch.float32).contiguous()
    n_out, c_in = w.shape[0], w.shape[1]
    ksize = w.shape[2] if w.ndim == 4 else 1
    e = epc(dtype)
    c_pad = _roundup(c_in, e) if c_pad is None else c_pad
    bk = block_k(dtype)
    k_pad = _roundup(ksize * ksize * c_pad, bk)
    n_pad = _roundup(n_out, 64)
    k_order = int(c_pad % bk == 0 and (c_split is None or c_split % bk == 0))
    out = torch.empty(n_pad, k_pad, dtype=dtype, device=w.device) if out is None else out
    L.check(L.load().mvldm_pack_weight(w.data_ptr(), out.data_ptr(), n_out, c_in, ksize, c_pad, n_pad, k_pad,
                                       int(geglu), k_order, dt(dtype), 0, 0, n_out, stream()))
    return PackedWeight(out, n_out, n_pad, k_pad, c_pad, ksize, geglu, k_order)


def pack_job(w: torch.Tensor, pw: PackedWeight, *, transpose: bool = False, c_off: int = 0) -> "L.PackJob":
    assert w.is_cuda and w.dtype == torch.float32 and w.is_contiguous()
    j = L.PackJob()
    j.src, j.dst = w.data_ptr(), pw.data.data_ptr()
    j.n_out, j.c_in, j.ksize = w.shape[0], w.shape[1], pw.ksize
    j.c_pad, j.n_pad, j.k_pad, j.geglu, j.k_order = pw.c_pad, pw.n_pad, pw.k_pad, int(pw.geglu), pw.k_order
    j.transpose, j.c_off, j.n_rows = int(transpose), c_off, (pw.n_out if transpose else w.shape[0])
    L.check(L.load().mvldm_pack_job_prepare(C.byref(j), dt(pw.data.dtype)))
    return j


class PackBatch:

    def __init__(self, jobs: Sequence["L.PackJob"], dtype: torch.dtype, device):
        self.n, self.dtype = len(jobs), dtype
        arr = (L.PackJob * max(len(jobs), 1))()
        b0 = 0
        for i, j in enumerate(jobs):
            C.memmove(C.byref(arr[i]), C.byref(j), C.sizeof(L.PackJob))
            arr[i].block0 = b0
            b0 += j.blocks
        self.total_blocks = b0
        raw = torch.frombuffer(bytearray(bytes(arr)), dtype=torch.uint8).clone()
        self.table = raw.to(device)
        self.block_job = None
        if jobs:
            self.block_job = torch.repeat_interleave(torch.arange(len(jobs), dtype=torch.int32), torch.tensor([j.blocks for j in jobs])).to(device)
            assert self.block_job.numel() == b0

    def run(self):
        L.check(L.load().mvldm_pack_weight_batch(self.table.data_ptr(), self.n, None if self.block_job is None else self.block_job.data_ptr(),
                                                 self.total_blocks, dt(self.dtype), stream()))


def conv_out_hw(h: int, w: int, ksize: int, stride: int, pad: int, upsample) -> tuple:
    if int(upsample) >= 2:
        return h, w
    hs, ws = (2 * h, 2 * w) if upsample else (h, w)
    if ksize == 3 and stride == 2 and pad == 0:
        return (hs + 1 - 3) // 2 + 1, (ws + 1 - 3) // 2 + 1
    return (hs + 2 * pad - ksize) // stride + 1, (ws + 2 * pad - ksize) // stride + 1


def use_skinny(d, pw: PackedWeight) -> torch.Tensor:
    t = pw.skinny()
    d.weight, d.k_order = ptr(t), 2
    return t


def igemm_desc(src0, src1, pw: PackedWeight, dst, *, n_img, h_in, w_in, h_out, w_out, stride=1, pad=None, upsample=False,
               bias=None, row_bias=None, residual=None, epilogue=L.EPI_NONE, out_scale=1.0, ws=None, splitk=0,
               tile=0, into=None) -> L.IgemmDesc:
    d = L.IgemmDesc() if into is None else into
    c0 = src0.shape[-1]
    c1 = 0 if src1 is None else src1.shape[-1]
    assert c0 + c1 == pw.c_pad, f"weight packed for {pw.c_pad} channels, sources give {c0}+{c1}"
    assert not pw.k_order or c0 % block_k(src0.dtype) == 0, "weight packed block-major but the source split is unaligned"
    d.src0, d.src1, d.weight = ptr(src0), ptr(src1), ptr(pw.data)
    d.bias, d.row_bias, d.residual, d.dst = ptr(bias), ptr(row_bias), ptr(residual), ptr(dst)
    d.c0, d.c1 = c0, c1
    d.n_img, d.h_in, d.w_in, d.h_out, d.w_out = n_img, h_in, w_in, h_out, w_out
    d.ksize, d.stride, d.upsample = pw.ksize, stride, int(upsample)
    d.pad = (pw.ksize // 2) if pad is None else pad
    d.n_out, d.n_pad, d.k_pad = pw.n_out, pw.n_pad, pw.k_pad
    d.row_bias_ld = 0 if row_bias is None else row_bias.stride(0)
    d.epilogue, d.act_dtype, d.dst_dtype = epilogue, dt(src0), dt(dst)
    d.splitk, d.tile, d.out_scale = splitk, tile, out_scale
    n_dst = pw.n_out // 2 if epilogue == L.EPI_GEGLU else pw.n_out
    d.dst_ld = 0 if dst.shape[-1] == n_dst else dst.shape[-1]
    d.k_order = pw.k_order
    if (tile & 63) == 15:
        use_skinny(d, pw)
    if ws is not None:
        d.workspace, d.workspace_bytes = ws.data_ptr(), ws.numel() * ws.element_size()
    else:
        d.workspace, d.workspace_bytes = None, 0
        if splitk == 0:
            d.splitk = 1
    return d


def conv2d(x: torch.Tensor, pw: PackedWeight, bias=None, *, x2=None, stride=1, pad=None, upsample=False, row_bias=None,
           residual=None, epilogue=L.EPI_NONE, out_dtype=None, out_scale=1.0, splitk=0, tile=0, out=None, dst=None) -> torch.Tensor:
    assert x.is_cuda and x.is_contiguous() and (x2 is None or x2.is_contiguous())
    n, h, w, _ = x.shape
    pad = (pw.ksize // 2) if pad is None else pad
    ho, wo = conv_out_hw(h, w, pw.ksize, stride, pad, upsample)
    n_dst = pw.n_out // 2 if epilogue == L.EPI_GEGLU else pw.n_out
    if dst is not None:
        up = 2 if int(upsample) >= 2 else 1
        assert out is None and dst.is_contiguous() and dst.dtype == (out_dtype or x.dtype) and dst.shape[-1] > n_dst
        assert dst.numel() == n * up * ho * up * wo * dst.shape[-1]
        out = dst
    elif out is None:
        out = torch.empty(n, ho, wo, n_dst, dtype=out_dtype or x.dtype, device=x.device)
    else:
        assert out.is_contiguous() and out.numel() == n * ho * wo * n_dst and out.dtype == (out_dtype or x.dtype)
        out = out.view(n, ho, wo, n_dst)
    scratch = None
    if splitk != 1:
        scratch = workspace(min(16 * n * ho * wo * pw.n_pad * 4, 256 << 20), x.device)
    d = igemm_desc(x, x2, pw, out, n_img=n, h_in=h, w_in=w, h_out=ho, w_out=wo, stride=stride, pad=pad,
                   upsample=upsample, bias=bias, row_bias=row_bias, residual=residual, epilogue=epilogue,
                   out_scale=out_scale, ws=scratch, splitk=splitk, tile=tile)
    L.check(L.load().mvldm_igemm_fwd(C.byref(d), stream()))
    return out


def upsample_phase_weights(w: torch.Tensor) -> list:
    assert w.ndim == 4 and w.shape[2:] == (3, 3)
    w = w.detach().to(torch.float32)
    rows = {0: (w[:, :, 0], w[:, :, 1] + w[:, :, 2]), 1: (w[:, :, 0] + w[:, :, 1], w[:, :, 2])}
    out = []
    for py in (0, 1):
        for px in (0, 1):
            taps = []
            for r in rows[py]:
                cols = (r[:, :, 0], r[:, :, 1] + r[:, :, 2]) if px == 0 else (r[:, :, 0] + r[:, :, 1], r[:, :, 2])
                taps.append(torch.stack(cols, dim=-1))
            out.append(torch.stack(taps, dim=-2).contiguous())
    return out


def conv2d_upsample_phases(x: torch.Tensor, pws, bias=None, tile=0, splitk=0) -> torch.Tensor:
    n, h, w, _ = x.shape
    out = torch.empty(n, 2 * h, 2 * w, pws[0].n_out, dtype=x.dtype, device=x.device)
    scratch = workspace(min(16 * n * h * w * pws[0].n_pad * 4, 256 << 20), x.device)
    for phase, pw in enumerate(pws):
        d = igemm_desc(x, None, pw, out, n_img=n, h_in=h, w_in=w, h_out=h, w_out=w, stride=1, pad=0, upsample=2 + phase,
                       bias=bias, splitk=splitk, tile=tile, ws=scratch)
        L.check(L.load().mvldm_igemm_fwd(C.byref(d), stream()))
    return out


def linear(x: torch.Tensor, pw: PackedWeight, bias=None, *, residual=None, epilogue=L.EPI_NONE, out_dtype=None,
           splitk=0, tile=0, out=None, dst=None) -> torch.Tensor:
    rows, c = x.shape
    y = conv2d(x.view(rows, 1, 1, c), pw, bias, residual=None if residual is None else residual.view(rows, 1, 1, -1),
               epilogue=epilogue, out_dtype=out_dtype, splitk=splitk, tile=tile, out=out, dst=None if dst is None else dst.view(rows, 1, 1, -1))
    return y.view(rows, -1)


def groupnorm(x: torch.Tensor, gamma, beta, groups: int, eps: float, silu: bool, x2=None, stats_out=None, out=None) -> torch.Tensor:
    assert x.is_cuda and x.is_contiguous() and (x2 is None or x2.is_contiguous())
    n, c0 = x.shape[0], x.shape[-1]
    c1 = 0 if x2 is None else x2.shape[-1]
    hw = math.prod(x.shape[1:-1])
    if out is None:
        y = torch.empty(*x.shape[:-1], c0 + c1, dtype=x.dtype, device=x.device)
    else:
        assert out.is_contiguous() and out.dtype == x.dtype and out.numel() == n * hw * (c0 + c1)
        y = out.view(*x.shape[:-1], c0 + c1)
    ws = workspace(max(n, 1) * L.GN_MAX_CHUNKS * groups * 2 * 8, x.device, "gn")
    L.check(L.load().mvldm_groupnorm_fwd(x.data_ptr(), ptr(x2), y.data_ptr(), gamma.data_ptr(), beta.data_ptr(), n, hw, c0, c1,
                                         groups, eps, int(silu), dt(x), ws.data_ptr(), ptr(stats_out), stream()))
    return y


def layernorm(x: torch.Tensor, gamma, beta, eps: float = 1e-5, out=None) -> torch.Tensor:
    assert x.is_cuda and x.is_contiguous()
    c = x.shape[-1]
    rows = x.numel() // c
    if out is None:
        y = torch.empty_like(x)
    else:
        assert out.is_contiguous() and out.dtype == x.dtype and out.numel() == x.numel()
        y = out.view(x.shape)
    L.check(L.load().mvldm_layernorm_fwd(x.data_ptr(), y.data_ptr(), gamma.data_ptr(), beta.data_ptr(), rows, c, eps,
                                         dt(x), stream()))
    return y


def make_segments(q_lens, kv_lens=None, device="cuda") -> torch.Tensor:
    kv_lens = q_lens if kv_lens is None else kv_lens
    rows, q0, k0 = [], 0, 0
    for ql, kl in zip(q_lens, kv_lens):
        rows.append([q0, ql, k0, kl])
        q0, k0 = q0 + ql, k0 + kl
    return torch.tensor(rows, dtype=torch.int32, device=device)


def attention(q: torch.Tensor, k: torch.Tensor, v: torch.Tensor, heads: int, head_dim: int, seg: torch.Tensor,
              max_q_len: int, scale: Optional[float] = None, lse: Optional[torch.Tensor] = None, out=None) -> torch.Tensor:
    assert q.is_cuda and q.stride(1) == 1 and k.stride(1) == 1 and v.stride(1) == 1
    if out is None:
        out = torch.empty(q.shape[0], heads * head_dim, dtype=q.dtype, device=q.device)
    assert out.stride(1) == 1 and out.dtype == q.dtype and out.shape[1] == heads * head_dim
    scale = head_dim ** -0.5 if scale is None else scale
    L.check(L.load().mvldm_attention_fwd(q.data_ptr(), k.data_ptr(), v.data_ptr(), out.data_ptr(), q.stride(0), k.stride(0),
                                         v.stride(0), out.stride(0), heads, head_dim, seg.data_ptr(), seg.shape[0],
                                         max_q_len, scale, dt(q), ptr(lse), 0 if lse is None else lse.stride(0), stream()))
    return out


def attention_merge(oa, lse_a, ob, lse_b, a_img, b_img, out_img, tokens: int, heads: int, head_dim: int, out=None) -> torch.Tensor:
    assert oa.is_cuda and oa.dtype == ob.dtype and oa.stride(1) == 1 and ob.stride(1) == 1
    assert all(t.dtype == torch.int32 and t.numel() == a_img.numel() for t in (a_img, b_img, out_img))
    if out is None:
        out = torch.empty(int(out_img.numel()) * tokens, heads * head_dim, dtype=oa.dtype, device=oa.device)
    assert out.stride(1) == 1 and out.dtype == oa.dtype
    L.check(L.load().mvldm_attention_merge(oa.data_ptr(), lse_a.data_ptr(), ob.data_ptr(), lse_b.data_ptr(), out.data_ptr(), a_img.data_ptr(),
                                           b_img.data_ptr(), out_img.data_ptr(), a_img.numel(), tokens, heads, head_dim, oa.stride(0), ob.stride(0),
                                           out.stride(0), lse_a.stride(0), lse_b.stride(0), dt(oa), stream()))
    return out


def gather_rows(src: torch.Tensor, dst: torch.Tensor, src_index=None, dst_index=None, n_rows: Optional[int] = None) -> torch.Tensor:
    assert src.is_cuda and src.is_contiguous() and dst.is_contiguous() and src.dim() == 2 and dst.dim() == 2
    row_bytes = src.shape[1] * src.element_size()
    assert row_bytes == dst.shape[1] * dst.element_size()
    for t in (src_index, dst_index):
        assert t is None or (t.dtype == torch.int32 and t.is_cuda and t.is_contiguous())
    if n_rows is None:
        n_rows = src_index.numel() if src_index is not None else dst_index.numel() if dst_index is not None else min(src.shape[0], dst.shape[0])
    L.check(L.load().mvldm_gather_rows(src.data_ptr(), dst.data_ptr(), ptr(src_index), ptr(dst_index), n_rows, row_bytes, stream()))
    return dst


def timestep_embed(timesteps: torch.Tensor, freqs: torch.Tensor, dim: int, flip_sin_to_cos: bool,
                   dtype=torch.float32) -> torch.Tensor:
    assert timesteps.dtype == torch.int64 and timesteps.is_cuda
    out = torch.empty(timesteps.numel(), dim, dtype=dtype, device=timesteps.device)
    L.check(L.load().mvldm_timestep_embed_fwd(timesteps.data_ptr(), freqs.data_ptr(), out.data_ptr(), timesteps.numel(),
                                              dim, int(flip_sin_to_cos), dt(dtype), stream()))
    return out


def eltwise(x: torch.Tensor, op: int, out_dtype=None) -> torch.Tensor:
    assert x.is_cuda and x.is_contiguous()
    y = torch.empty(x.shape, dtype=out_dtype or x.dtype, device=x.device)
    L.check(L.load().mvldm_eltwise_fwd(x.data_ptr(), y.data_ptr(), x.numel(), op, dt(x), dt(y), stream()))
    return y


def silu(x, out_dtype=None):
    return eltwise(x, L.ELT_SILU, out_dtype)


def convert(x, out_dtype):
    return eltwise(x, L.ELT_COPY, out_dtype)


def nchw_to_nhwc(src: torch.Tensor, dtype, dst: Optional[torch.Tensor] = None, c_off: int = 0,
                 dst_c: Optional[int] = None, scale: float = 1.0, shift: float = 0.0,
                 img_map: Optional[torch.Tensor] = None) -> torch.Tensor:
    assert src.is_cuda and src.dtype == torch.float32 and src.is_contiguous()
    n, c, h, w = src.shape
    if dst is None:
        dst_c = c if dst_c is None else dst_c
        dst = torch.zeros(n, h, w, dst_c, dtype=dtype, device=src.device)
    L.check(L.load().mvldm_nchw_to_nhwc(src.data_ptr(), dst.data_ptr(), n, c, h * w, dst.shape[-1], c_off, dt(dst), scale, shift,
                                        ptr(img_map), stream()))
    return dst
# ... 670 lines not shown
```

mv_ldm_amd/plan.py:

```python
from __future__ import annotations

import ctypes as C
import json
import os
import sys
from dataclasses import dataclass
from typing import List, Optional

import torch

from . import _lib as L
from .ops import PackedWeight, conv_out_hw, dt, igemm_desc, ptr, use_skinny


def _PIN_TILE() -> int:
    v = os.environ.get("MVLDM_IGEMM_TILE")
    return int(v) if v else 0


@dataclass
class OpMeta:
    name: str
    kind: int
    flops: float = 0.0
# ... 299 lines not shown
        self._emit(op, name, 0.0, 0.0, (step_ptr, t_table, timesteps, tgt_rows))

    def memcpy(self, dst, src, name="memcpy"):
        assert dst.is_contiguous() and src.is_contiguous() and dst.numel() * dst.element_size() == src.numel() * src.element_size()
        op = L.Op()
        op.kind = L.OP_MEMCPY
        op.u.memcpy_.src, op.u.memcpy_.dst, op.u.memcpy_.bytes = ptr(src), ptr(dst), src.numel() * src.element_size()
        self._emit(op, name, 0.0, 2.0 * src.numel() * src.element_size(), (dst, src))

    def gather_rows(self, src, dst, src_index=None, dst_index=None, n_rows=None, name="gather_rows"):
        idx = src_index if src_index is not None else dst_index
        n = int(n_rows if n_rows is not None else (idx.numel() if idx is not None else dst.shape[0]))
        row_bytes = dst[0].numel() * dst.element_size()
        assert src[0].numel() * src.element_size() == row_bytes and row_bytes % 16 == 0 and dst.is_contiguous() and src.is_contiguous()
        assert all(i is None or (i.dtype == torch.int32 and i.numel() == n) for i in (src_index, dst_index))
        assert (src_index is not None or src.shape[0] >= n) and (dst_index is not None or dst.shape[0] >= n)
        op = L.Op()
        op.kind = L.OP_GATHER_ROWS
        g = op.u.gather
        g.src, g.dst, g.src_index, g.dst_index, g.row_bytes, g.n_rows = ptr(src), ptr(dst), ptr(src_index), ptr(dst_index), row_bytes, n
        self._emit(op, name, 0.0, 2.0 * n * row_bytes, (src, dst, src_index, dst_index))

    def nhwc_to_nchw(self, src, dst, c=None, c_off=0, scale=1.0, shift=0.0, clamp01=False, name="nhwc_to_nchw"):
        n, h, w, sc = src.shape
        op = L.Op()
        op.kind = L.OP_NHWC_TO_NCHW
        l = op.u.layout
        l.src, l.dst, l.n_img, l.c, l.hw, l.other_c, l.other_c_off, l.dtype = ptr(src), ptr(dst), n, c or sc, h * w, sc, c_off, dt(src)
        l.clamp01, l.scale, l.shift = int(clamp01), scale, shift
        self._emit(op, name, 0.0, src.numel() * src.element_size() + dst.numel() * 4, (src, dst))
        return dst

    def nchw_to_nhwc(self, src, dst, c_off=0, scale=1.0, shift=0.0, img_map=None, name="nchw_to_nhwc"):
        n, c, h, w = src.shape
        op = L.Op()
        op.kind = L.OP_NCHW_TO_NHWC
        l = op.u.layout
        l.src, l.dst, l.n_img, l.c, l.hw, l.other_c, l.other_c_off, l.dtype = ptr(src), ptr(dst), n, c, h * w, dst.shape[-1], c_off, dt(dst)
        l.scale, l.shift, l.img_map = scale, shift, ptr(img_map)
        self._emit(op, name, 0.0, src.numel() * 4 + src.numel() * dst.element_size(), (src, dst, img_map))
        return dst

    def ray_encode(self, extr, intr, h, w, out_nhwc, c_off, img_map=None, out_nchw=None, name="ray_encode", mode=0, n_origin_octaves=0,
                   n_dir_octaves=0, plucker=False):
        op = L.Op()
        op.kind = L.OP_RAY_ENCODE
        r = op.u.rays
        r.extrinsics, r.intrinsics, r.out_nchw, r.out_nhwc, r.img_map = ptr(extr), ptr(intr), ptr(out_nchw), ptr(out_nhwc), ptr(img_map)
        r.n_cam, r.h, r.w = extr.shape[0], h, w
        r.nhwc_c, r.nhwc_c_off, r.nhwc_dtype = (0, 0, L.F32) if out_nhwc is None else (out_nhwc.shape[-1], c_off, dt(out_nhwc))
        r.mode, r.n_origin_octaves, r.n_dir_octaves, r.plucker = mode, n_origin_octaves, n_dir_octaves, int(plucker)
        self._emit(op, name, 0.0, extr.shape[0] * h * w * 6 * 4.0, (extr, intr, out_nhwc, out_nchw, img_map))

    def posterior_sample(self, moments, noise, out, scale=1.0, name="posterior_sample"):
        n, c2, h, w = moments.shape
        op = L.Op()
        op.kind = L.OP_POSTERIOR_SAMPLE
        q = op.u.posterior
        q.moments, q.noise, q.out, q.n, q.c, q.hw, q.scale = ptr(moments), ptr(noise), ptr(out), n, c2 // 2, h * w, scale
        self._emit(op, name, 0.0, moments.numel() * 4 * 2.0, (moments, noise, out))
        return out

    def finalize(self, autotune: Optional[bool] = None) -> "Plan":
        assert self.record
        if autotune is None:
            autotune = os.environ.get("MVLDM_AUTOTUNE", "1") != "0"
        if autotune and torch.device(self.device).type == "cuda":
            autotune_igemm(self.ops, srcs=self.__dict__.get("_tune_srcs"), skinny=self._skinny_pw, keep=self.keep)
            autotune_wgrad(self.ops)
            if type(self) is Builder and _BATCH_SPLIT:
                self.ops, self.meta = autosplit_igemm(self.ops, self.meta, skinny=self._skinny_pw, keep=self.keep)
        return Plan(self.ops, self.meta, self.keep, self.device)


_TUNE_CACHE = {}
_WGRAD_CACHE = {}
_SPLIT_CACHE = {}
_VALIDATED = set()
_TUNE_TILES = tuple(int(t) for t in os.environ["MVLDM_TUNE_TILES"].split(",")) if os.environ.get("MVLDM_TUNE_TILES") else (0, 1, 2, 3, 4, 5, 6, 7, 8, 9, 10, 11, 12, 13, 14)


def tune_cache_state() -> dict:
    return {"version": 2, "igemm": {json.dumps(list(k)): (int(v) if isinstance(v, int) else list(v)) for k, v in _TUNE_CACHE.items()},
            "wgrad": {json.dumps(list(k)): int(v) for k, v in _WGRAD_CACHE.items()},
            "split": {json.dumps(list(k)): int(v) for k, v in _SPLIT_CACHE.items()}}


def set_tune_cache_state(state: dict, replace: bool = False) -> None:
    if replace:
        _TUNE_CACHE.clear()
        _WGRAD_CACHE.clear()
        _SPLIT_CACHE.clear()
    for name, cache in (("igemm", _TUNE_CACHE), ("wgrad", _WGRAD_CACHE), ("split", _SPLIT_CACHE)):
        for k, v in (state.get(name) or {}).items():
            cache[tuple(json.loads(k))] = int(v) if isinstance(v, int) else list(v)


def save_tune_cache(path: Optional[str] = None) -> Optional[str]:
    path = path or os.environ.get("MVLDM_TUNE_CACHE")
    if not path:
        return None
    tmp = f"{path}.{os.getpid()}.tmp"
    with open(tmp, "w") as f:
        json.dump(tune_cache_state(), f, indent=0, sort_keys=True)
    os.replace(tmp, path)
    return path


def load_tune_cache(path: Optional[str] = None) -> int:
    path = path or os.environ.get("MVLDM_TUNE_CACHE")
    if not path or not os.path.exists(path):
        return 0
    with open(path) as f:
        set_tune_cache_state(json.load(f))
    return len(_TUNE_CACHE) + len(_WGRAD_CACHE) + len(_SPLIT_CACHE)


def broadcast_tune_cache(dist, src: int = 0, device=None) -> None:
    box = [tune_cache_state() if dist.get_rank() == src else None]
    dist.broadcast_object_list(box, src=src, device=device)
    set_tune_cache_state(box[0], replace=True)


load_tune_cache()


def _igemm_signature(d) -> tuple:
    return (d.n_img, d.h_in, d.w_in, d.h_out, d.w_out, d.c0, d.c1, d.ksize, d.stride, d.pad, d.upsample, d.n_out, d.n_pad,
            d.k_pad, d.epilogue, d.act_dtype, d.dst_dtype, d.k_order, d.dst_ld, bool(d.residual), bool(d.row_bias),
            bool(d.bias), d.splitk, d.workspace_bytes)


_SMALL_ROWS = int(os.environ.get("MVLDM_TUNE_SMALL_ROWS", "64"))
_SPLITS = (0, 1, 2, 4, 8, 16, 32)
_MID_ROWS = int(os.environ.get("MVLDM_TUNE_MID_ROWS", "40000"))
_MID_SPLITS = (0, 1, 2, 3, 4, 6, 8)
_SMALL_TILES = tuple(int(t) for t in os.environ.get("MVLDM_TUNE_SMALL_TILES", "0,1,2,3,4,5").split(","))


_SKINNY = os.environ.get("MVLDM_SKINNY", "1") != "0"
_SKINNY_ROWS = int(os.environ.get("MVLDM_SKINNY_ROWS", "2304"))
_SKINNY_CFGS = tuple(int(c) for c in os.environ.get("MVLDM_SKINNY_CFGS", "0,1,2,5,6,7,8,9,10,12,13,18,19,20,38,39,40,41,42,43,44,46").split(","))


def skinny_rule(rows: int, n_pad: int) -> bool:
    if os.environ.get("MVLDM_AUTOTUNE", "1") != "0" or os.environ.get("MVLDM_SKINNY_RULE", "1") == "0":
        return False
    return rows <= 160 or (rows <= 1152 and n_pad <= 1280)


def skinny_candidate(pw: PackedWeight, rows: int, c0: int, c1: int, upsample, dtype) -> bool:
    return (_SKINNY and dtype != torch.float32 and rows <= _SKINNY_ROWS and not (upsample is True or upsample == 1) and pw.can_skinny()
            and c0 % 64 == 0 and c1 % 64 == 0)


def _unpack_choice(v):
    return (int(v), None) if isinstance(v, int) else (int(v[0]), None if v[1] is None else int(v[1]))


_TUNE_COLD = int(os.environ.get("MVLDM_TUNE_COLD", "9216"))
_THRASH = []
_THRASH_FILLS = [0]


def _thrash(device=None):
    if not _THRASH or (device is not None and _THRASH[0].device != torch.device(device)):
        _THRASH[:] = [torch.empty(640 << 20, dtype=torch.uint8, device=torch.cuda.current_device() if device is None else device)]
    return _THRASH[0]


def autotune_igemm(ops, min_rows: int = 2048, iters: int = 4, srcs=None, skinny=None, keep=None) -> int:
    lib = L.load()
    stream = torch.cuda.current_stream().cuda_stream
    e0, e1 = torch.cuda.Event(enable_timing=True), torch.cuda.Event(enable_timing=True)
    timed = 0
    tune_dev = next((t.device for pair in (srcs or {}).values() for t in pair if t is not None), None)
    if srcs:
        seen, gen = set(), None
        for pair in srcs.values():
            for t in pair:
                if t is not None and t.is_floating_point() and t.data_ptr() not in seen:
                    seen.add(t.data_ptr())
                    if gen is None:
                        gen = torch.Generator(device=t.device)
                        gen.manual_seed(0x5EED)
                    t.normal_(generator=gen)
    for idx, op in enumerate(ops):
        if op.kind != L.OP_IGEMM:
            continue
        d = op.u.igemm
        rows = d.n_img * d.h_out * d.w_out
        sk_pw = (skinny or {}).get(idx)
        if d.tile != 0 or d.act_dtype == L.F32 or d.k_order != 1 or (rows < min(min_rows, _SMALL_ROWS) and sk_pw is None):
            continue
        small = rows < min_rows
        key = _igemm_signature(d) + (("sk",) if sk_pw is not None else ())
        best = _TUNE_CACHE.get(key)
        if best is not None and (_unpack_choice(best)[0] & 63) not in (set(_TUNE_TILES) | set(_SMALL_TILES) | {17, 19} | ({15} if sk_pw is not None else set())):
            best = None
        if best is None:
            trial = L.Op()
            C.memmove(C.byref(trial), C.byref(op), C.sizeof(L.Op))
            can_split = small and bool(d.workspace) and d.splitk == 0
            mid = (not small) and rows < _MID_ROWS and bool(d.workspace) and d.splitk == 0
            cands = [(t, sk) for t in _TUNE_TILES for sk in _MID_SPLITS] if mid else [(t, None) for t in _TUNE_TILES] if not small else \
                    [(t, sk) for t in _SMALL_TILES if t in _TUNE_TILES or not os.environ.get("MVLDM_TUNE_TILES") for sk in (_SPLITS if can_split else (None,))]
            n_it = iters if not small else 3 * iters
            cold = _TUNE_COLD > 0 and rows <= _TUNE_COLD
            if not small and 17 not in _TUNE_TILES and not os.environ.get("MVLDM_TUNE_TILES") and d.ksize == 3 and d.stride == 1 \
                    and d.src1 is None and not d.upsample and d.w_in <= 24:
                cands = cands + [(17, None)]
            if not small and d.ksize == 1 and not os.environ.get("MVLDM_TUNE_TILES"):
                cands = cands + [(19, None), (13 | (1 << 13), None)]
            if sk_pw is not None:
                cands = cands + [(15 | (c << 8), 1) for c in _SKINNY_CFGS]
            results = []
            for tile, sk in cands:
                trial.u.igemm.tile = tile
                trial.u.igemm.splitk = d.splitk if sk is None else sk
                trial.u.igemm.weight, trial.u.igemm.k_order = d.weight, d.k_order
                if (tile & 63) == 15:
                    use_skinny(trial.u.igemm, sk_pw)
                if lib.mvldm_op_run(C.byref(trial), stream) != 0:
                    continue
                if cold:
                    t_sum = 0.0
                    for _ in range(n_it):
                        _thrash(tune_dev).zero_()
                        _THRASH_FILLS[0] += 1
                        e0.record()
                        lib.mvldm_op_run(C.byref(trial), stream)
                        e1.record()
                        e1.synchronize()
                        t_sum += e0.elapsed_time(e1)
                    results.append((t_sum, tile, sk))
                    continue
                e0.record()
                for _ in range(n_it):
                    lib.mvldm_op_run(C.byref(trial), stream)
                e1.record()
                e1.synchronize()
                results.append((e0.elapsed_time(e1), tile, sk))
            t_rule = next(t for t, tile, sk in results if tile == 0 and sk in (None, 0))
            t_best, tile_best, sk_best = min(results, key=lambda r: r[0])
            best = [tile_best, sk_best] if t_best < 0.97 * t_rule else [0, None]
            _TUNE_CACHE[key] = best
            _VALIDATED.add(key)
            timed += 1
        tile, sk = _unpack_choice(best)
        if tile != 0 and key not in _VALIDATED:
            trial = L.Op()
            C.memmove(C.byref(trial), C.byref(op), C.sizeof(L.Op))
            trial.u.igemm.tile = tile
            if sk is not None:
                trial.u.igemm.splitk = sk
            if (tile & 63) == 15:
                if sk_pw is None:
                    tile, sk = 0, None
                else:
                    use_skinny(trial.u.igemm, sk_pw)
            if tile != 0 and lib.mvldm_op_run(C.byref(trial), stream) != 0:
                tile, sk = 0, None
                _TUNE_CACHE[key] = [0, None]
            _VALIDATED.add(key)
        d.tile = tile
        if sk is not None:
            d.splitk = sk
        if (tile & 63) == 15:
            t = use_skinny(d, sk_pw)
            sk_pw._skinny_pinned = True
            if keep is not None:
                keep.append(t)
        elif sk_pw is not None:
            sk_pw.drop_skinny()
    if timed:
        save_tune_cache()
        _THRASH.clear()
    return timed


_BATCH_SPLIT = os.environ.get("MVLDM_BATCH_SPLIT", "1") != "0"
_SPLIT_MIN_ROWS = int(os.environ.get("MVLDM_BATCH_SPLIT_MIN_ROWS", "16384"))


def _split_candidates(d) -> list:
    rpi = d.h_out * d.w_out
    rows = d.n_img * rpi
    out = []
    for bn in (320, 256):
        n_tiles = -(-d.n_pad // bn)
        m_tiles = -(-rows // 256)
        if m_tiles * n_tiles <= 256 or (m_tiles * n_tiles) % 256 == 0 or (m_tiles * n_tiles) % 256 > 216:
            continue
        for m1 in range(m_tiles - 1, 0, -1):
            if (m1 * n_tiles) % 256 == 0 and (m1 * 256) % rpi == 0:
                n1 = m1 * 256 // rpi
                frac = 1.0 - n1 / d.n_img
                if 0.03 <= frac <= 0.45 and n1 not in out:
                    out.append(n1)
                break
    return out


def _image_range(op, i0: int, n: int):
    q = L.Op()
    C.memmove(C.byref(q), C.byref(op), C.sizeof(L.Op))
    d = q.u.igemm
    es = 4 if d.act_dtype == L.F32 else 2
    ds = 4 if d.dst_dtype == L.F32 else 2
    n_dst = d.n_out // 2 if d.epilogue == L.EPI_GEGLU else d.n_out
    px_in, px_out = d.h_in * d.w_in, d.h_out * d.w_out

    def off(p, nbytes):
        return (p + nbytes) if p else p
    d.src0 = off(d.src0, i0 * px_in * d.c0 * es)
    d.src1 = off(d.src1, i0 * px_in * d.c1 * es)
    d.dst = off(d.dst, i0 * px_out * (d.dst_ld or n_dst) * ds)
    d.residual = off(d.residual, i0 * px_out * n_dst * es)
    d.row_bias = off(d.row_bias, i0 * d.row_bias_ld * 4)
    d.n_img = n
    d.tile, d.splitk = 0, 0
    return q


def _time_ops(ops, iters: int) -> float:
    lib = L.load()
    stream = torch.cuda.current_stream().cuda_stream
    e0, e1 = torch.cuda.Event(enable_timing=True), torch.cuda.Event(enable_timing=True)
    for o in ops:
        L.check(lib.mvldm_op_run(C.byref(o), stream))
    e0.record()
    for _ in range(iters):
        for o in ops:
            lib.mvldm_op_run(C.byref(o), stream)
    e1.record()
    e1.synchronize()
    return e0.elapsed_time(e1) / iters


def autosplit_igemm(ops, meta, skinny=None, keep=None, iters: int = 6):
    new_ops, new_meta, decided = [], [], 0
    for idx, (op, m) in enumerate(zip(ops, meta)):
        d = op.u.igemm if op.kind == L.OP_IGEMM else None
        rows = d.n_img * d.h_out * d.w_out if d is not None else 0
        ok = (d is not None and rows >= _SPLIT_MIN_ROWS and d.act_dtype != L.F32 and d.k_order == 1 and d.stride == 1 and not d.upsample
              and (d.tile & 63) != 15 and not _PIN_TILE() and bool(d.workspace) and idx not in (skinny or {}))
        n1 = 0
        if ok:
            key = _igemm_signature(d)[:-2] + (d.workspace_bytes,)
            if key in _SPLIT_CACHE:
                n1 = _SPLIT_CACHE[key]
            else:
                best_t, t_whole = None, None
                for cand in _split_candidates(d):
                    parts = [_image_range(op, 0, cand), _image_range(op, cand, d.n_img - cand)]
                    try:
                        autotune_igemm(parts, iters=4)
                        if t_whole is None:
                            t_whole = _time_ops([op], iters)
                        t = _time_ops(parts, iters)
                    except L.MvldmError:
                        continue
                    if os.environ.get("MVLDM_BATCH_SPLIT_LOG"):
                        print(f"[batch split] {m.name}: {d.n_img} images x {d.h_out}x{d.w_out}, N {d.n_out}, K {d.k_pad}: whole {t_whole * 1e3:.1f} us (tile {d.tile & 63}, "
                              f"splitk {d.splitk}); {cand} + {d.n_img - cand}: {t * 1e3:.1f} us (tiles {parts[0].u.igemm.tile & 63} / {parts[1].u.igemm.tile & 63}, "
                              f"splitk {parts[1].u.igemm.splitk})", file=sys.stderr, flush=True)
                    if t < 0.97 * t_whole and (best_t is None or t < best_t):
                        best_t, n1 = t, cand
                _SPLIT_CACHE[key] = n1
                decided += 1
        if n1:
            parts = [_image_range(op, 0, n1), _image_range(op, n1, d.n_img - n1)]
            autotune_igemm(parts, iters=4)
            for k, (q, i0, cnt) in enumerate(zip(parts, (0, n1), (n1, d.n_img - n1))):
                q.tag = len(new_ops)
                new_ops.append(q)
                share = cnt / d.n_img
                new_meta.append(OpMeta(m.name if k == 0 else m.name + "[rest]", m.kind, m.flops * share, m.bytes * share))
        else:
            op.tag = len(new_ops)
            new_ops.append(op)
            new_meta.append(m)
    if decided:
        save_tune_cache()
    return new_ops, new_meta


_WGRAD_TARGETS = tuple(int(t) for t in os.environ.get("MVLDM_TUNE_WGRAD_TARGETS", "0,1,2,3,4,5").split(","))


def autotune_wgrad(ops, iters: int = 3) -> int:
    lib = L.load()
    stream = torch.cuda.current_stream().cuda_stream
    e0, e1 = torch.cuda.Event(enable_timing=True), torch.cuda.Event(enable_timing=True)
    timed = 0
    scratch = None
    for op in ops:
        if op.kind != L.OP_WGRAD:
            continue
        d = op.u.wgrad
        if d.act_dtype == L.F32 or (d.accumulate >> 8) & 3:
            continue
        key = (d.c0, d.c1, d.n_img, d.h_in, d.w_in, d.h_out, d.w_out, d.ksize, d.stride, d.pad, d.upsample, d.n_out, d.dy_ld, d.act_dtype,
               int(d.workspace_bytes), d.accumulate & 1)
        best = _WGRAD_CACHE.get(key)
        if best is None:
            trial = L.Op()
            C.memmove(C.byref(trial), C.byref(op), C.sizeof(L.Op))
            need = d.n_out * d.c_in * d.ksize * d.ksize
            if scratch is None or scratch.numel() < need:
                scratch = torch.zeros(need, dtype=torch.float32, device=torch.cuda.current_device())
            else:
                scratch[:need].zero_()
            trial.u.wgrad.grad = scratch.data_ptr()
            results = []
            for form in (1, 2):
                for tcode in _WGRAD_TARGETS:
                    v = form + 4 * tcode
                    trial.u.wgrad.accumulate = (d.accumulate & 1) | (v << 8)
                    if lib.mvldm_op_run(C.byref(trial), stream) != 0:
                        break
                    e0.record()
                    for _ in range(iters):
                        lib.mvldm_op_run(C.byref(trial), stream)
                    e1.record()
                    e1.synchronize()
                    results.append((e0.elapsed_time(e1), v))
            best = min(results)[1] if results else 0
            _WGRAD_CACHE[key] = best
            timed += 1
        d.accumulate = (d.accumulate & 1) | (best << 8)
    if timed:
        save_tune_cache()
    return timed


class Plan:

    def __init__(self, ops, meta, keep, device):
        self.meta, self._keep, self.device = list(meta), list(keep), device
        self.ops = list(ops)
        self.tiles = [int(op.u.igemm.tile) if op.kind == L.OP_IGEMM else None for op in ops]
        arr = (L.Op * max(len(ops), 1))(*ops)
        h = C.c_void_p()
        L.check(L.load().mvldm_plan_create(arr, len(ops), C.byref(h)))
        self._h = h
        self._stream = None
        self.captured = False

    def __len__(self):
        return len(self.meta)

    @staticmethod
    def _cur():
        return torch.cuda.current_stream().cuda_stream

    def run(self, first: int = 0, last: Optional[int] = None):
        last = len(self.meta) if last is None else last
        L.check(L.load().mvldm_plan_run_range(self._h, first, last, self._cur()))

    def capture(self):
        if self._stream is None:
            self._stream = torch.cuda.Stream(device=self.device)
        self._stream.wait_stream(torch.cuda.current_stream())
        L.check(L.load().mvldm_plan_capture(self._h, self._stream.cuda_stream))
        torch.cuda.current_stream().wait_stream(self._stream)
        self.captured = True

    def replay(self):
        L.check(L.load().mvldm_plan_replay(self._h, self._cur()))

    def profile(self, iters: int = 3):
        out = (C.c_float * max(len(self.meta), 1))()
        L.check(L.load().mvldm_plan_profile(self._h, self._cur(), iters, out))
        return [float(v) for v in out[:len(self.meta)]]

    def __del__(self):
        try:
            if getattr(self, "_h", None):
                L.load().mvldm_plan_destroy(self._h)
                self._h = None
        except Exception:
            pass
```

Before: 49.76.

## Add stream-K scheduling for tile-10 implicit GEMM with fixup reduction

Adds a stream-K variant of the 256x320 tile-10 implicit-GEMM kernel. Each workgroup takes a contiguous range of (tile, k-block) units, so work spreads evenly across CUs when the tile count is not a multiple of the CU count. Tiles split across workgroups write fp32 partials to a workspace, and a separate fixup kernel sums them and applies bias, activation, residual and store. The autotuner offers stream-K as a candidate, so it only runs where it is timed faster. In exchange it adds workspace traffic, an extra kernel launch, and looping control flow inside the main kernel.

```diff
diff --git a/include/mvldm.h b/include/mvldm.h
--- a/include/mvldm.h
+++ b/include/mvldm.h
@@ -47,6 +47,7 @@
     float out_scale;
     size_t workspace_bytes;
 } mvldm_igemm_desc;
+#define MVLDM_TILE_STREAMK (1 << 15)
 int mvldm_igemm_fwd(const mvldm_igemm_desc* d, mvldm_stream_t stream);
 size_t mvldm_igemm_workspace_bytes(const mvldm_igemm_desc* d);
 
diff --git a/mv_ldm_amd/_build.py b/mv_ldm_amd/_build.py
--- a/mv_ldm_amd/_build.py
+++ b/mv_ldm_amd/_build.py
@@ -10,7 +10,7 @@
 
 CSRC = Path(__file__).resolve().parent / "csrc"
 LIB = CSRC / "libmvldm_hip.so"
-SOURCES = ["api.cpp", "plan.cpp", "igemm.hip", "igemm_small.hip", "igemm_large.hip", "igemm_xl.hip", "igemm_halo.hip", "pack.hip", "attention.hip", "norm.hip", "misc.hip",
+SOURCES = ["api.cpp", "plan.cpp", "igemm.hip", "igemm_small.hip", "igemm_large.hip", "igemm_xl.hip", "igemm_sk.hip", "igemm_halo.hip", "pack.hip", "attention.hip", "norm.hip", "misc.hip",
            "wgrad.hip", "attention_bwd.hip", "norm_bwd.hip", "train_misc.hip", "linear_pp.hip", "linear_pw.hip", "linear_ws.hip", "linear_rs.hip", "skinny.hip", "metrics.hip", "lpips.hip", "dists.hip", "fid.hip", "inception.hip", "kid.hip", "cropshim.hip", "jpeg.hip", "jpeg_host.cpp"]
 HEADERS = [*sorted(CSRC.glob("*.h")), CSRC.parent.parent / "include" / "mvldm.h"]
 FLAGS = ["--offload-arch=gfx950", "-O3", "-std=c++17", "-fPIC", "-ffp-contract=off", "-Wno-unused-result",
diff --git a/mv_ldm_amd/_lib.py b/mv_ldm_amd/_lib.py
--- a/mv_ldm_amd/_lib.py
+++ b/mv_ldm_amd/_lib.py
@@ -12,6 +12,9 @@
 ELT_COPY, ELT_SILU, ELT_GELU = 0, 1, 2
 NORM_BWD_STORE = 0x100
 GN_MAX_CHUNKS = 32
+TILE_STREAMK = 1 << 15
+TILE10_STREAMK = 10 | TILE_STREAMK
+ERR_ARG, ERR_HIP, ERR_UNSUPPORTED = -1, -2, -3
 JPEG_GRAY, JPEG_444, JPEG_422, JPEG_420 = 0, 1, 2, 3
 JPEG_REASONS = ("ok", "not a JPEG", "truncated", "corrupt", "progressive", "frame type", "precision", "components", "sampling", "colour space",
                 "scans", "size", "range guard")
diff --git a/mv_ldm_amd/csrc/igemm.hip b/mv_ldm_amd/csrc/igemm.hip
--- a/mv_ldm_amd/csrc/igemm.hip
+++ b/mv_ldm_amd/csrc/igemm.hip
@@ -3,6 +3,7 @@
 #include <cstdlib>
 
 #include "igemm_common.h"
+#include "linear_common.h"
 
 namespace mvldm {
 
@@ -35,6 +36,83 @@
     }
 }
 
+__device__ __forceinline__ void reduce_act8(const IgemmParams& p, int m, int col, float (&a)[8]) {
+    if (p.bias) {
+#pragma unroll
+        for (int e = 0; e < 8; ++e) a[e] += p.bias[col + e];
+    }
+    if (p.row_bias) {
+        const float* rb = p.row_bias + (size_t)(m / p.hw_out) * p.row_bias_ld + col;
+#pragma unroll
+        for (int e = 0; e < 8; ++e) a[e] += rb[e];
+    }
+    if (p.epilogue == MVLDM_EPI_SILU) {
+#pragma unroll
+        for (int e = 0; e < 8; ++e) a[e] = silu_f(a[e]);
+    } else if (p.epilogue == MVLDM_EPI_GELU) {
+#pragma unroll
+        for (int e = 0; e < 8; ++e) a[e] = gelu_erf_fast(a[e]);
+    }
+}
+template <typename T> __device__ __forceinline__ void reduce_store8(const IgemmParams& p, int m, int col, float (&a)[8]) {
+#pragma unroll
+    for (int e = 0; e < 8; ++e) a[e] *= p.out_scale;
+    if (p.residual) {
+        const Chunk<T> rc = load_chunk<T>(reinterpret_cast<const T*>(p.residual) + (size_t)m * p.n_dst + col);
+#pragma unroll
+        for (int e = 0; e < 8; ++e) a[e] += rc.get(e);
+    }
+    size_t drow = (size_t)m;
+    if (p.scatter) {
+        const int img = m / p.hw_out, rem = m - img * p.hw_out;
+        const int i = rem / p.w_out, j = rem - i * p.w_out;
+        drow = ((size_t)img * (2 * p.h_out) + 2 * i + p.ph_y) * (size_t)(2 * p.w_out) + 2 * j + p.ph_x;
+    }
+    Chunk<T> oc;
+#pragma unroll
+    for (int e = 0; e < 8; ++e) oc.set(e, a[e]);
+    store_chunk<T>(reinterpret_cast<T*>(p.dst) + drow * p.dst_ld + col, oc);
+}
+
+constexpr int kSkFixBlocks = 8;
+template <typename T, int BM, int BN> __global__ __launch_bounds__(256) void igemm_streamk_fixup(const IgemmParams p) {
+    constexpr int ROWS = BM / kSkFixBlocks, CPR = BN / 8;
+    const int s = blockIdx.x / kSkFixBlocks, band = blockIdx.x - s * kSkFixBlocks;
+    const int n_t = sk_contributors(p.sk_blocks, p.tiles_m * p.tiles_n * p.sk_blocks, p.sk_wgs, s);
+    if (n_t <= 1) return;
+    int tm, tn;
+    sk_tile(sk_grid(p), s, tm, tn);
+    const int units = p.tiles_m * p.tiles_n * p.sk_blocks;
+    for (int e = threadIdx.x; e < ROWS * CPR; e += 256) {
+        const int row = band * ROWS + e / CPR, cc = (e % CPR) * 8;
+        const int m = tm * BM + row, col = tn * BN + cc;
+        if (m >= p.M || col >= p.n_dst) continue;
+        const float* w0 = p.ws + row * BN + cc;
+        float a[8];
+#pragma unroll
+        for (int k = 0; k < 8; ++k) a[k] = 0.f;
+        int c = 0;
+        for (; c + 2 <= n_t; c += 2) {
+            const float* w1 = w0 + (size_t)sk_slot(p.sk_blocks, units, p.sk_wgs, s, c) * (BM * BN);
+            const float* w2 = w0 + (size_t)sk_slot(p.sk_blocks, units, p.sk_wgs, s, c + 1) * (BM * BN);
+            const f32x4 l0 = *reinterpret_cast<const f32x4*>(w1), h0 = *reinterpret_cast<const f32x4*>(w1 + 4);
+            const f32x4 l1 = *reinterpret_cast<const f32x4*>(w2), h1 = *reinterpret_cast<const f32x4*>(w2 + 4);
+#pragma unroll
+            for (int k = 0; k < 4; ++k) { a[k] += l0[k]; a[4 + k] += h0[k]; }
+#pragma unroll
+            for (int k = 0; k < 4; ++k) { a[k] += l1[k]; a[4 + k] += h1[k]; }
+        }
+        if (c < n_t) {
+            const float* w1 = w0 + (size_t)sk_slot(p.sk_blocks, units, p.sk_wgs, s, c) * (BM * BN);
+            const f32x4 l0 = *reinterpret_cast<const f32x4*>(w1), h0 = *reinterpret_cast<const f32x4*>(w1 + 4);
+#pragma unroll
+            for (int k = 0; k < 4; ++k) { a[k] += l0[k]; a[4 + k] += h0[k]; }
+        }
+        reduce_act8(p, m, col, a);
+        reduce_store8<T>(p, m, col, a);
+    }
+}
+
 template <typename T> __global__ __launch_bounds__(256) void igemm_splitk_reduce_vec(const IgemmParams p) {
     const bool geglu = p.epilogue == MVLDM_EPI_GEGLU;
     const int cpr = p.n_dst / 8;
@@ -79,44 +157,17 @@
                 for (int e = 0; e < 4; ++e) { g[e] += gl[e]; g[4 + e] += gh[e]; }
             }
         }
-        if (p.bias) {
-#pragma unroll
-            for (int e = 0; e < 8; ++e) a[e] += p.bias[col + e];
-        }
         if (geglu) {
+            if (p.bias) {
+#pragma unroll
+                for (int e = 0; e < 8; ++e) a[e] += p.bias[col + e];
+            }
 #pragma unroll
             for (int e = 0; e < 8; ++e) a[e] *= gelu_erf_fast(g[e] + (p.bias ? p.bias[p.n_dst + col + e] : 0.f));
         } else {
-            if (p.row_bias) {
-                const float* rb = p.row_bias + (size_t)(m / p.hw_out) * p.row_bias_ld + col;
-#pragma unroll
-                for (int e = 0; e < 8; ++e) a[e] += rb[e];
-            }
-            if (p.epilogue == MVLDM_EPI_SILU) {
-#pragma unroll
-                for (int e = 0; e < 8; ++e) a[e] = silu_f(a[e]);
-            } else if (p.epilogue == MVLDM_EPI_GELU) {
-#pragma unroll
-                for (int e = 0; e < 8; ++e) a[e] = gelu_erf_fast(a[e]);
-            }
-        }
-#pragma unroll
-        for (int e = 0; e < 8; ++e) a[e] *= p.out_scale;
-        if (p.residual) {
-            const Chunk<T> rc = load_chunk<T>(reinterpret_cast<const T*>(p.residual) + (size_t)m * p.n_dst + col);
-#pragma unroll
-            for (int e = 0; e < 8; ++e) a[e] += rc.get(e);
-        }
-        size_t drow = (size_t)m;
-        if (p.scatter) {
-            const int img = m / p.hw_out, rem = m - img * p.hw_out;
-            const int i = rem / p.w_out, j = rem - i * p.w_out;
-            drow = ((size_t)img * (2 * p.h_out) + 2 * i + p.ph_y) * (size_t)(2 * p.w_out) + 2 * j + p.ph_x;
-        }
-        Chunk<T> oc;
-#pragma unroll
-        for (int e = 0; e < 8; ++e) oc.set(e, a[e]);
-        store_chunk<T>(reinterpret_cast<T*>(p.dst) + drow * p.dst_ld + col, oc);
+            reduce_act8(p, m, col, a);
+        }
+        reduce_store8<T>(p, m, col, a);
     }
 }
 
@@ -133,7 +184,22 @@
 
 static thread_local int t_force_sync = 0;
 
+static bool accepts_tile10(const mvldm_igemm_desc& d) {
+    return d.act_dtype != MVLDM_F32 && d.k_order == 1 && d.dst_dtype != MVLDM_F32 && d.n_pad % 320 == 0 && d.epilogue != MVLDM_EPI_GEGLU &&
+           d.upsample != 1 && d.n_out % 8 == 0 && (d.dst_ld <= 0 || d.dst_ld % 8 == 0) && !(d.ksize == 3 && d.src1);
+}
+
+struct SkShape { int wgs, blocks, tiles; };
+static SkShape sk_shape(const mvldm_igemm_desc& d) {
+    const int M = d.n_img * d.h_out * d.w_out, taps = d.ksize * d.ksize;
+    return {d.splitk > 1 ? d.splitk : cu_count(), std::max(1, d.k_pad / 64 / std::max(taps, 1)), cdiv(M, kTiles[10].bm) * cdiv(d.n_pad, kTiles[10].bn)};
+}
+static size_t sk_workspace_bytes(const SkShape& k) {
+    return (size_t)sk_slots(k.tiles * k.blocks, k.wgs) * kTiles[10].bm * kTiles[10].bn * sizeof(float);
+}
+
 static int launch_igemm(const IgemmParams& p, int tile, int act_dtype, hipStream_t s) {
+    if (p.sk_wgs) return igemm_launch_sk(p, tile, act_dtype, s);
     if (tile >= 1 && tile <= 5) return igemm_launch_small(p, tile, act_dtype, s);
     if (tile >= 6 && tile <= 8) return igemm_launch_large(p, tile, act_dtype, s);
     if (tile == 9 || tile == 10 || tile == 18) return igemm_launch_xl(p, tile, act_dtype, s);
@@ -145,9 +211,7 @@
 static void choose_config(const mvldm_igemm_desc& d, int M, int k_tiles, int& tile, int& splitk, size_t ws_bytes) {
     const int target = kEnvTarget ? kEnvTarget : 512;
     if (tile == 0) {
-        const bool can10 = d.act_dtype != MVLDM_F32 && d.k_order == 1 && d.dst_dtype != MVLDM_F32 && d.n_pad % 320 == 0 &&
-                           d.epilogue != MVLDM_EPI_GEGLU && d.upsample != 1 && d.n_out % 8 == 0 && (d.dst_ld <= 0 || d.dst_ld % 8 == 0) &&
-                           !(d.ksize == 3 && d.src1);
+        const bool can10 = accepts_tile10(d);
         const int wgs10 = cdiv(M, 256) * (d.n_pad / 320);
         const double eff10 = (double)wgs10 / (256.0 * cdiv(wgs10, 256));
         if (can10 && (wgs10 >= 1024 || (wgs10 >= 512 && (eff10 >= 0.9 || d.ksize == 1)))) tile = 10;
@@ -175,6 +239,10 @@
     const int epc = d.act_dtype == MVLDM_F32 ? 4 : 8;
     const int bk = d.act_dtype == MVLDM_F32 ? 32 : 64;
     MVLDM_REQUIRE(d.src0 && d.weight && d.dst, "igemm: null pointer");
+    const bool sk = (d.tile & MVLDM_TILE_STREAMK) != 0;
+    if (sk && !((d.tile & 63) == 10 && accepts_tile10(d) && !d.src1 && d.c1 == 0 && d.splitk >= 0))
+        return set_error(MVLDM_ERR_UNSUPPORTED, "igemm: stream-K takes tile 10 on 16-bit block-major one-source 1x1 / 3x3 / 2x2 phase convs "
+                                                "(n_pad a multiple of 320, 8-aligned 16-bit output, no GEGLU)");
     const bool phase = d.upsample >= 2;
     MVLDM_REQUIRE(d.upsample >= 0 && d.upsample <= 5, "igemm: upsample %d", d.upsample);
     MVLDM_REQUIRE(phase ? (d.ksize == 2 && d.stride == 1 && d.h_out == d.h_in && d.w_out == d.w_in && !d.src1 && !d.residual &&
@@ -210,7 +278,7 @@
     tile = d.tile & 63;
     t_force_sync = (d.tile >> 12) & 1;
     const int force_px = (d.tile >> 8) & 15;
-    int splitk = d.splitk;
+    int splitk = sk ? 1 : d.splitk;
     MVLDM_REQUIRE(((tile >= 0 && tile <= kNumTiles) || tile == 17 || deep_tile(tile)) && splitk >= 0, "igemm: tile/splitk");
     choose_config(d, p.M, p.k_tiles, tile, splitk, d.workspace_bytes);
     if (splitk > 1)
@@ -264,8 +332,23 @@
         MVLDM_REQUIRE(p.ty0 + p.cy >= 0 && p.tx0 + p.cx >= 0 && hc < d.h_in && wc < d.w_in,
                       "igemm: conv geometry (pad %d, stride %d) not supported", d.pad, d.stride);
     }
+    if (sk && !(tile == 10 && p.use_bl && p.stage_epi && p.splitk == 1))
+        return set_error(MVLDM_ERR_UNSUPPORTED, "igemm: stream-K needs the lean 16-bit loop and the staged epilogue");
     p.tiles_m = cdiv(p.M, kTiles[tile].bm);
     p.tiles_n = cdiv(d.n_pad, kTiles[tile].bn);
+    p.sk_wgs = p.sk_blocks = 0;
+    if (sk) {
+        const SkShape k = sk_shape(d);
+        p.sk_wgs = k.wgs; p.sk_blocks = p.k_tiles / p.taps;
+        MVLDM_REQUIRE(p.sk_blocks == k.blocks && p.tiles_m * p.tiles_n == k.tiles && (double)k.tiles * k.blocks < 1.0e9, "igemm: stream-K units");
+        int slabs = 0;
+        for (int t = 0; t < k.tiles; ++t) slabs = std::max(slabs, sk_contributors(k.blocks, k.tiles * k.blocks, k.wgs, t));
+        if (slabs > 1)
+            MVLDM_REQUIRE(d.workspace && ((uintptr_t)d.workspace % 16) == 0 && sk_workspace_bytes(k) <= d.workspace_bytes,
+                          "igemm: stream-K workspace too small (%d slots of a tile)", sk_slots(k.tiles * k.blocks, k.wgs));
+        MVLDM_REQUIRE(((uintptr_t)d.dst % 16) == 0 && (!d.residual || ((uintptr_t)d.residual % 16) == 0), "igemm: stream-K needs 16-byte aligned rows");
+        p.splitk = slabs > 1 ? slabs : 1;
+    }
     p.korder = d.k_order;
     if (d.k_order)
         MVLDM_REQUIRE(d.k_order == 1 && p.ctot % bk == 0 && d.c0 % bk == 0 && d.k_pad == p.taps * p.ctot,
@@ -325,6 +408,15 @@
         using T = decltype(t);
         int r = launch_igemm(p, tile, Elt<T>::DT, s);
         if (r) return r;
+        if (p.sk_wgs) {
+            if constexpr (sizeof(T) == 2) {
+                if (p.splitk > 1) {
+                    hipLaunchKernelGGL((igemm_streamk_fixup<T, kTiles[10].bm, kTiles[10].bn>), dim3((unsigned)(p.tiles_m * p.tiles_n * kSkFixBlocks)), dim3(256), 0, s, p);
+                    return check_launch();
+                }
+            }
+            return (int)MVLDM_OK;
+        }
         if (p.splitk > 1) {
             if constexpr (sizeof(T) == 2) {
                 if (!p.dst_f32 && p.n_dst % 8 == 0 && p.dst_ld % 8 == 0 && ((uintptr_t)p.ws % 16) == 0 &&
@@ -356,5 +448,6 @@
 extern "C" size_t mvldm_igemm_workspace_bytes(const mvldm_igemm_desc* d) {
     if (!d) return 0;
     const size_t M = (size_t)d->n_img * d->h_out * d->w_out;
+    if ((d->tile & MVLDM_TILE_STREAMK) && M > 0) return sk_workspace_bytes(sk_shape(*d));
     return (size_t)16 * M * d->n_pad * sizeof(float);
 }
diff --git a/mv_ldm_amd/csrc/igemm_bl.h b/mv_ldm_amd/csrc/igemm_bl.h
--- a/mv_ldm_amd/csrc/igemm_bl.h
+++ b/mv_ldm_amd/csrc/igemm_bl.h
@@ -207,7 +207,7 @@
     }
 }
 
-template <typename T, int BM, int BN, int WM, int WN, int KS, bool DUAL, int STAGES, bool UPS>
+template <typename T, int BM, int BN, int WM, int WN, int KS, bool DUAL, int STAGES, bool UPS, bool SK = false>
 __global__ __launch_bounds__(WM* WN * 64) void igemm_bl_kernel(const IgemmParams p) {
     using M_ = Mma<T>;
     static_assert(sizeof(T) == 2, "16-bit activation types only");
@@ -220,13 +220,33 @@
     static_assert(STAGES >= 2 && STAGES <= 8, "ring depth");
     extern __shared__ __attribute__((aligned(16))) char smem[];
 
-    const auto [lane, wave, wm, wn, hi, l31] = wave_lane<WN>();
-    int split, tm, tn;
-    if (!map_block(p, split, tm, tn)) return;
-    const int cb0 = split * (p.k_tiles_per_split / TAPS);
-    const int cb1 = min(cb0 + p.k_tiles_per_split / TAPS, p.k_tiles / TAPS);
-
+    const WaveLane wl0 = wave_lane<WN>();
+    int split, tm, tn, cb0, cb1;
+    [[maybe_unused]] int sk_units = 0, sk_r = 0, sk_u0 = 0, sk_u = 0, sk_end = 0;
+    [[maybe_unused]] bool sk_partial = false;
+    if constexpr (SK) {
+        static_assert(NW == 8 && STAGES == 2 && TM * TN > 8 && !DUAL && !UPS, "stream-K: the 8-wave simple loop, one source");
+        sk_units = p.tiles_m * p.tiles_n * p.sk_blocks;
+        sk_r = sk_rank(p.sk_wgs, (int)blockIdx.x);
+        sk_u = sk_u0 = sk_begin(sk_units, p.sk_wgs, sk_r);
+        sk_end = sk_begin(sk_units, p.sk_wgs, sk_r + 1);
+        if (sk_u >= sk_end) return;
+    } else {
+        if (!map_block(p, split, tm, tn)) return;
+        cb0 = split * (p.k_tiles_per_split / TAPS);
+        cb1 = min(cb0 + p.k_tiles_per_split / TAPS, p.k_tiles / TAPS);
+    }
+    do {
+    int lane_ = wl0.lane;
+    if constexpr (SK) asm volatile("" : "+v"(lane_));
+    const int lane = lane_, wave = wl0.wave, wm = wl0.wm, wn = wl0.wn, hi = lane >> 5, l31 = lane & 31;
     const int slot = lane & 7, rsub = lane >> 3;
+    if constexpr (SK) {
+        const SkSegment seg = sk_segment(p.sk_blocks, sk_units, p.sk_wgs, sk_r, sk_u0, sk_u, sk_end);
+        sk_tile(sk_grid(p), seg.tile, tm, tn);
+        cb0 = seg.cb0; cb1 = seg.cb1; split = seg.slot; sk_partial = !seg.direct;
+        sk_u += cb1 - cb0;
+    }
     BlAddr<TAPS, A_IT, DUAL, UPS> ad;
 #pragma unroll
     for (int it = 0; it < A_IT; ++it) {
@@ -431,12 +451,23 @@
 #undef MVLDM_BL_ISSUE
 #undef MVLDM_BL_ISSUE_R
     asm volatile("s_waitcnt vmcnt(0)" ::: "memory");
-    if constexpr (TM * TN > 4) {
+    if constexpr (SK) {
+        IgemmParams q = p;
+        if (sk_partial) {
+            q.ws = p.ws + (size_t)split * (BM * BN);
+            q.M = min(BM, p.M - tm * BM);
+            q.n_pad = BN;
+        }
+        igemm_epilogue_staged_sk<T, BM, BN, WM, WN>(q, acc, sk_partial ? 0 : tm, sk_partial ? 0 : tn, wm, wn, wave, lane, smem, sk_partial);
+        if (sk_u >= sk_end) break;
+        __syncthreads();
+    } else if constexpr (TM * TN > 4) {
         igemm_epilogue_staged<T, BM, BN, WM, WN>(p, acc, tm, tn, split, wm, wn, wave, lane, smem);
     } else {
         if (p.stage_epi) igemm_epilogue_staged<T, BM, BN, WM, WN>(p, acc, tm, tn, split, wm, wn, wave, lane, smem);
         else igemm_epilogue<T, BM, BN, WM, WN>(p, acc, tm, tn, split, wm, wn, hi, l31);
     }
+    } while (SK);
 }
 
 template <typename T, int BM, int BN, int WM, int WN> static int launch_sync(const IgemmParams& p, hipStream_t s) {
@@ -446,12 +477,12 @@
                          8 * p.sub_m * p.sub_n * p.splitk, WM * WN * 64, p, s);
 }
 
-template <typename T, int BM, int BN, int WM, int WN, int KS, bool DUAL, int STAGES, bool UPS>
+template <typename T, int BM, int BN, int WM, int WN, int KS, bool DUAL, int STAGES, bool UPS, bool SK = false>
 static int launch_bl_s(const IgemmParams& p, hipStream_t s) {
     static std::atomic<uint64_t> done{0};
     constexpr int ring = STAGES * (BM + BN) * 128, park = WM * WN * 32 * (park_blocks(BN / WN / 32) * 32 + 4) * 4;
-    return launch_kernel(igemm_bl_kernel<T, BM, BN, WM, WN, KS, DUAL, STAGES, UPS>, done, ring > park ? ring : park,
-                         8 * p.sub_m * p.sub_n * p.splitk, WM * WN * 64, p, s);
+    return launch_kernel(igemm_bl_kernel<T, BM, BN, WM, WN, KS, DUAL, STAGES, UPS, SK>, done, ring > park ? ring : park,
+                         SK ? p.sk_wgs : 8 * p.sub_m * p.sub_n * p.splitk, WM * WN * 64, p, s);
 }
 template <typename T, int BM, int BN, int WM, int WN, int KS, bool DUAL, int DEPTH = 0>
 static int launch_bl(const IgemmParams& p, hipStream_t s) {
@@ -489,6 +520,14 @@
     return dual ? launch_bl<T, BM, BN, WM, WN, 1, true>(p, s) : launch_bl<T, BM, BN, WM, WN, 1, false>(p, s);
 }
 
+template <typename T, int BM, int BN, int WM, int WN> static int launch_bl_sk(const IgemmParams& p, hipStream_t s) {
+    if (p.c1 > 0 || p.upsample || !p.stage_epi || p.sk_wgs < 1)
+        return set_error(MVLDM_ERR_UNSUPPORTED, "igemm: stream-K takes one-source 1x1 / 3x3 / 2x2 phase convs with the staged epilogue");
+    if (p.ksize == 2) return launch_bl_s<T, BM, BN, WM, WN, 2, false, 2, false, true>(p, s);
+    if (p.ksize == 3) return launch_bl_s<T, BM, BN, WM, WN, 3, false, 2, false, true>(p, s);
+    return launch_bl_s<T, BM, BN, WM, WN, 1, false, 2, false, true>(p, s);
+}
+
 template <typename T, int BM, int BN, int WM, int WN> static int launch_tile(const IgemmParams& p, hipStream_t s) {
     if constexpr (sizeof(T) == 2) {
         if (p.use_bl) return launch_bl_any<T, BM, BN, WM, WN>(p, s);
diff --git a/mv_ldm_amd/csrc/igemm_common.h b/mv_ldm_amd/csrc/igemm_common.h
--- a/mv_ldm_amd/csrc/igemm_common.h
+++ b/mv_ldm_amd/csrc/igemm_common.h
@@ -2,6 +2,7 @@
 #include <algorithm>
 
 #include "common.h"
+#include "streamk.h"
 
 namespace mvldm {
 
@@ -27,6 +28,7 @@
     unsigned src0_bytes, src1_bytes, w_bytes;
     int use_bl, stage_epi;
     int nt_store;
+    int sk_wgs, sk_blocks;
 };
 
 template <typename T> struct Mma;
@@ -350,6 +352,18 @@
     igemm_epilogue_rowblock<T, BM, BN, WM, WN, 0>(p, acc, st, tm, tn, split, wm, wn, mode, lane);
 }
 
+template <typename T, int BM, int BN, int WM, int WN>
+__device__ __forceinline__ void igemm_epilogue_staged_sk(const IgemmParams& p, f32x16 (&acc)[BM / WM / 32][BN / WN / 32], int tm, int tn,
+                                                         int wm, int wn, int wave, int lane, char* smem, bool partial) {
+    constexpr int PITCH = park_blocks(BN / WN / 32) * 32 + 4;
+    float* st = reinterpret_cast<float*>(smem) + wave * (32 * PITCH);
+    const int mode = partial ? EPI_PARTIAL : (p.epilogue == MVLDM_EPI_SILU ? EPI_ACT_SILU : (p.epilogue == MVLDM_EPI_GELU ? EPI_ACT_GELU : EPI_PLAIN));
+    __syncthreads();
+    igemm_epilogue_rowblock<T, BM, BN, WM, WN, 0>(p, acc, st, tm, tn, 0, wm, wn, mode, lane);
+}
+
+__host__ __device__ __forceinline__ SkGrid sk_grid(const IgemmParams& p) { return SkGrid{p.tiles_m, p.tiles_n, p.px, p.sub_m, p.sub_n, p.grp_m, p.grp_n, p.m_fast}; }
+
 struct WaveLane { int lane, wave, wm, wn, hi, l31; };
 template <int WN> __device__ __forceinline__ WaveLane wave_lane() {
     const int tid = threadIdx.x, lane = tid & 63;
@@ -419,5 +433,6 @@
 int igemm_launch_large(const IgemmParams& p, int tile, int act_dtype, hipStream_t s);
 int igemm_launch_xl(const IgemmParams& p, int tile, int act_dtype, hipStream_t s);
 int igemm_launch_halo(const IgemmParams& p, int tile, int act_dtype, hipStream_t s);
-
-}
+int igemm_launch_sk(const IgemmParams& p, int tile, int act_dtype, hipStream_t s);
+
+}
diff --git a/mv_ldm_amd/csrc/igemm_sk.hip b/mv_ldm_amd/csrc/igemm_sk.hip
--- /dev/null
+++ b/mv_ldm_amd/csrc/igemm_sk.hip
@@ -0,0 +1,14 @@
+#include "igemm_bl.h"
+
+namespace mvldm {
+
+int igemm_launch_sk(const IgemmParams& p, int tile, int act_dtype, hipStream_t s) {
+    if (tile != 10) return set_error(MVLDM_ERR_UNSUPPORTED, "igemm: stream-K is built for tile 10 (asked: tile %d)", tile);
+    if (int rc = require_bl(p, tile, act_dtype)) return rc;
+    return dispatch_16bit(act_dtype, [&](auto t) {
+        using T = decltype(t);
+        return launch_bl_sk<T, 256, 320, 4, 2>(p, s);
+    });
+}
+
+}
diff --git a/mv_ldm_amd/csrc/streamk.h b/mv_ldm_amd/csrc/streamk.h
--- /dev/null
+++ b/mv_ldm_amd/csrc/streamk.h
@@ -0,0 +1,88 @@
+#pragma once
+
+#if defined(__HIPCC__)
+#define MVLDM_SK_FN __host__ __device__ __forceinline__
+#else
+#define MVLDM_SK_FN inline
+#endif
+
+namespace mvldm {
+
+MVLDM_SK_FN int sk_begin(int units, int wgs, int r) {
+    const int q = units / wgs, rem = units - q * wgs;
+    return r * q + (r < rem ? r : rem);
+}
+
+MVLDM_SK_FN int sk_owner(int units, int wgs, int u) {
+    const int q = units / wgs, rem = units - q * wgs;
+    const int big = rem * (q + 1);
+    return u < big ? u / (q + 1) : rem + (u - big) / q;
+}
+
+MVLDM_SK_FN int sk_contributors(int blocks, int units, int wgs, int s) {
+    return sk_owner(units, wgs, (s + 1) * blocks - 1) - sk_owner(units, wgs, s * blocks) + 1;
+}
+
+struct SkSegment {
+    int tile, cb0, cb1;
+    int slab;
+    int slot;
+    bool direct;
+};
+
+MVLDM_SK_FN SkSegment sk_segment(int blocks, int units, int wgs, int r, int u_begin, int u, int u_end) {
+    SkSegment g;
+    g.tile = u / blocks;
+    g.cb0 = u - g.tile * blocks;
+    const int left = u_end - u;
+    g.cb1 = g.cb0 + left < blocks ? g.cb0 + left : blocks;
+    g.direct = g.cb0 == 0 && g.cb1 == blocks;
+    g.slab = r - sk_owner(units, wgs, g.tile * blocks);
+    g.slot = 2 * r + (u > u_begin ? 1 : 0);
+    return g;
+}
+
+MVLDM_SK_FN int sk_slot(int blocks, int units, int wgs, int s, int c) {
+    const int r = sk_owner(units, wgs, s * blocks) + c;
+    return 2 * r + (sk_begin(units, wgs, r) < s * blocks ? 1 : 0);
+}
+
+MVLDM_SK_FN int sk_slots(int units, int wgs) { return 2 * (wgs < units ? wgs : units); }
+
+MVLDM_SK_FN int sk_rank(int wgs, int g) {
+    const int x = g & 7;
+    int before = 0;
+    for (int i = 0; i < x; ++i) before += (wgs - i + 7) / 8;
+    return before + (g >> 3);
+}
+
+struct SkGrid { int tiles_m, tiles_n, px, sub_m, sub_n, grp_m, grp_n, m_fast; };
+
+MVLDM_SK_FN void sk_tile(const SkGrid& g, int s, int& tm, int& tn) {
+    tm = tn = 0;
+    for (int xcd = 0; xcd < 8; ++xcd) {
+        const int xm = xcd % g.px, xn = xcd / g.px;
+        int vm = g.tiles_m - xm * g.sub_m, vn = g.tiles_n - xn * g.sub_n;
+        vm = vm < 0 ? 0 : (vm > g.sub_m ? g.sub_m : vm);
+        vn = vn < 0 ? 0 : (vn > g.sub_n ? g.sub_n : vn);
+        const int cnt = vm * vn;
+        if (s >= cnt) { s -= cnt; continue; }
+        int tml, tnl;
+        if (g.grp_m * g.grp_n > 1) {
+            const int gm = g.grp_m, gn = g.grp_n;
+            const int nfull = vm / gm, per_super = gm * vn;
+            int mg, gm_eff, rr;
+            if (s < nfull * per_super) { mg = s / per_super; rr = s - mg * per_super; gm_eff = gm; }
+            else { mg = nfull; rr = s - nfull * per_super; gm_eff = vm - nfull * gm; }
+            const int ng = rr / (gm_eff * gn), r2 = rr - ng * gm_eff * gn;
+            tnl = ng * gn + r2 / gm_eff;
+            tml = mg * gm + r2 % gm_eff;
+        } else if (g.m_fast) { tnl = s / vm; tml = s - tnl * vm; }
+        else { tml = s / vn; tnl = s - tml * vn; }
+        tm = xm * g.sub_m + tml;
+        tn = xn * g.sub_n + tnl;
+        return;
+    }
+}
+
+}
diff --git a/mv_ldm_amd/ops.py b/mv_ldm_amd/ops.py
--- a/mv_ldm_amd/ops.py
+++ b/mv_ldm_amd/ops.py
@@ -215,7 +215,10 @@
         assert out.is_contiguous() and out.numel() == n * ho * wo * n_dst and out.dtype == (out_dtype or x.dtype)
         out = out.view(n, ho, wo, n_dst)
     scratch = None
-    if splitk != 1:
+    if tile & L.TILE_STREAMK:
+        q = igemm_desc(x, x2, pw, out, n_img=n, h_in=h, w_in=w, h_out=ho, w_out=wo, stride=stride, pad=pad, upsample=upsample, splitk=splitk, tile=tile)
+        scratch = workspace(max(int(L.load().mvldm_igemm_workspace_bytes(C.byref(q))), 16), x.device)
+    elif splitk != 1:
         scratch = workspace(min(16 * n * ho * wo * pw.n_pad * 4, 256 << 20), x.device)
     d = igemm_desc(x, x2, pw, out, n_img=n, h_in=h, w_in=w, h_out=ho, w_out=wo, stride=stride, pad=pad,
                    upsample=upsample, bias=bias, row_bias=row_bias, residual=residual, epilogue=epilogue,
diff --git a/mv_ldm_amd/plan.py b/mv_ldm_amd/plan.py
--- a/mv_ldm_amd/plan.py
+++ b/mv_ldm_amd/plan.py
@@ -475,6 +475,30 @@
 def skinny_candidate(pw: PackedWeight, rows: int, c0: int, c1: int, upsample, dtype) -> bool:
     return (_SKINNY and dtype != torch.float32 and rows <= _SKINNY_ROWS and not (upsample is True or upsample == 1) and pw.can_skinny()
             and c0 % 64 == 0 and c1 % 64 == 0)
+
+
+_STREAMK = os.environ.get("MVLDM_STREAMK", "1") != "0"
+_CU_COUNT = []
+
+
+def _cu_count() -> int:
+    if not _CU_COUNT:
+        n = C.c_int(0)
+        L.load().mvldm_device_info(C.byref(n), None, None, 0)
+        _CU_COUNT.append(n.value if n.value > 0 else 256)
+    return _CU_COUNT[0]
+
+
+def streamk_candidate(d) -> bool:
+    if not _STREAMK or d.act_dtype == L.F32 or d.dst_dtype == L.F32 or d.k_order != 1 or d.n_pad % 320 or d.src1 or d.epilogue == L.EPI_GEGLU \
+            or d.upsample == 1 or d.n_out % 8 or (d.dst_ld > 0 and d.dst_ld % 8) or not d.workspace:
+        return False
+    tiles = -(-(d.n_img * d.h_out * d.w_out) // 256) * (d.n_pad // 320)
+    return tiles % _cu_count() != 0
+
+
+def is_streamk(tile: int) -> bool:
+    return bool(tile & L.TILE_STREAMK)
 
 
 def _unpack_choice(v):
@@ -535,6 +559,8 @@
                 cands = cands + [(17, None)]
             if not small and d.ksize == 1 and not os.environ.get("MVLDM_TUNE_TILES"):
                 cands = cands + [(19, None), (13 | (1 << 13), None)]
+            if not small and streamk_candidate(d) and (10 in _TUNE_TILES or not os.environ.get("MVLDM_TUNE_TILES")):
+                cands = cands + [(L.TILE10_STREAMK, 0)]
             if sk_pw is not None:
                 cands = cands + [(15 | (c << 8), 1) for c in _SKINNY_CFGS]
             results = []
@@ -667,7 +693,7 @@
         d = op.u.igemm if op.kind == L.OP_IGEMM else None
         rows = d.n_img * d.h_out * d.w_out if d is not None else 0
         ok = (d is not None and rows >= _SPLIT_MIN_ROWS and d.act_dtype != L.F32 and d.k_order == 1 and d.stride == 1 and not d.upsample
-              and (d.tile & 63) != 15 and not _PIN_TILE() and bool(d.workspace) and idx not in (skinny or {}))
+              and (d.tile & 63) != 15 and not is_streamk(d.tile) and not _PIN_TILE() and bool(d.workspace) and idx not in (skinny or {}))
         n1 = 0
         if ok:
             key = _igemm_signature(d)[:-2] + (d.workspace_bytes,)
```

New measurement: 49.93, median of 6. About the same (+0.4%).
